# salesforce/LayoutDETR

Measured on AMD Instinct MI355X. Metric: images/sec G+D fwd-bwd, 256x256 bg x9 elems, higher is better.
Workload: dtype f32

## Files before the change

### include/ldetr_hip.h

```cpp
#ifndef LDETR_HIP_H
#define LDETR_HIP_H

#include <stdint.h>

#ifdef __cplusplus
extern "C" {
#endif

const char* ldetr_last_error(void);
int ldetr_abi_version(void);

int ldetr_debug_trace_tiles(int64_t* buffer);

int ldetr_set_split_bf16(int tiles);

int ldetr_engine_launch_counts(int64_t* f32_pipe, int64_t* bf16_split_pipe);

int ldetr_set_workspace(void* ptr, int64_t bytes);

typedef struct ldetr_tensor4 {
    int N, C, H, W;
    int64_t sn, sc, sh, sw;
} ldetr_tensor4;

typedef struct ldetr_epilogue {
    float alpha;
    const float* col_scale;
    const float* col_bias;
    const float* samp_scale;
    int64_t samp_ld;
    const float* residual;
    int64_t ldr;
    int act;
    float act_alpha;
    float act_gain;
    const float* mask_src;
    int64_t ldm;
    int mask_mode;
    float out_scale;
    float p_drop;
    uint64_t seed;
    const uint64_t* seed_ptr;
    int accumulate;
    float* a_rowsum;
} ldetr_epilogue;

int ldetr_bias_act_f32(const float* x, const float* b, const float* xref, const float* yref, const float* dy, float* y,
                       int64_t sizeX, int sizeB, int64_t stepB, int grad, int act, float alpha, float gain, float clamp,
                       void* stream);

int ldetr_upfirdn2d_f32(const float* x, const float* f, float* y, int N, int C, int inH, int inW,
                        const int64_t* x_strides_nchw, int fh, int fw, int64_t f_stride_h, int64_t f_stride_w,
                        int upx, int upy, int downx, int downy, int padx0, int padx1, int pady0, int pady1, int flip,
                        float gain, int outH, int outW, const int64_t* y_strides_nchw,
                        const float* act_bias, int has_act, float act_alpha, float act_gain, void* stream);

int ldetr_gemm_f32(const float* A, int64_t lda, int ta, const float* B, int64_t ldb, int tb, float* C, int64_t ldc,
                   int M, int N, int K, int splitk, const ldetr_epilogue* ep, int pix_per_sample, void* stream);

typedef struct ldetr_gemm_desc {
    const float* A; int64_t lda; int ta;
    const float* B; int64_t ldb; int tb;
    float* C; int64_t ldc;
    int M, N, K, splitk;
    const ldetr_epilogue* ep;
    int pix_per_sample;
} ldetr_gemm_desc;
int ldetr_gemm_pair_f32(const ldetr_gemm_desc* g0, const ldetr_gemm_desc* g1, void* stream);
int ldetr_gemm_pair_is_single_launch(const ldetr_gemm_desc* g0, const ldetr_gemm_desc* g1);

int ldetr_conv2d_fwd_f32(const float* x, const ldetr_tensor4* xt, const float* w, int Cout, int KH, int KW, int stride,
                         int pad, float* y, int64_t ldy, int OH, int OW, const float* in_scale, int64_t in_scale_ld,
                         const ldetr_epilogue* ep, void* stream);
int ldetr_conv2d_bwd_data_f32(const float* dy, const ldetr_tensor4* dyt, const float* w, int Cin, int KH, int KW,
                              int stride, int pad, float* dx, int64_t lddx, int IH, int IW, const float* dy_scale,
                              int64_t dy_scale_ld, const ldetr_epilogue* ep, void* stream);
int ldetr_conv2d_bwd_weight_f32(const float* x, const ldetr_tensor4* xt, const float* dy, const ldetr_tensor4* dyt,
                                float* dw, int KH, int KW, int stride, int pad, int splitk, const float* x_scale,
                                int64_t x_scale_ld, const float* dy_scale, int64_t dy_scale_ld, int accumulate, void* stream);

int ldetr_conv_transpose2d_fwd_f32(const float* x, const ldetr_tensor4* xt, const float* w, int Cout, int KH, int KW,
                                   int stride, int pad, float* y, int64_t ldy, int OH, int OW, const float* in_scale,
                                   int64_t in_scale_ld, const ldetr_epilogue* ep, void* stream);
int ldetr_conv_transpose2d_bwd_data_f32(const float* dy, const ldetr_tensor4* dyt, const float* w, int Cin, int KH,
                                        int KW, int stride, int pad, float* dx, int64_t lddx, int IH, int IW,
                                        const float* dy_scale, int64_t dy_scale_ld, const ldetr_epilogue* ep,
                                        void* stream);
int ldetr_conv_transpose2d_bwd_weight_f32(const float* x, const ldetr_tensor4* xt, const float* dy,
                                          const ldetr_tensor4* dyt, float* dw, int KH, int KW, int stride, int pad,
                                          int splitk, const float* x_scale, int64_t x_scale_ld, const float* dy_scale,
                                          int64_t dy_scale_ld, int accumulate, void* stream);

int ldetr_attention_fwd_f32(const float* q, int64_t ldq, const float* k, int64_t ldk, const float* v, int64_t ldv,
                            const unsigned char* key_padding_mask, float* out, int64_t ldo, float* lse, int B, int H,
                            int Lq, int Lk, int head_dim, float scale, float p_drop, uint64_t seed, const uint64_t* seed_ptr,
                            int causal, void* stream);
int ldetr_attention_bwd_f32(const float* q, int64_t ldq, const float* k, int64_t ldk, const float* v, int64_t ldv,
                            const unsigned char* key_padding_mask, const float* out, int64_t ldo, const float* lse,
                            const float* dout, int64_t lddo, float* dq, int64_t lddq, float* dk, int64_t lddk,
                            float* dv, int64_t lddv, int B, int H, int Lq, int Lk, int head_dim, float scale,
                            float p_drop, uint64_t seed, const uint64_t* seed_ptr, int causal, void* stream);

int ldetr_torgb_bwd_finish_f32(const float* dws, const float* s, const float* w, int B, int C, float* dw, float* ds, void* stream);

int ldetr_loss_combine_fwd_f32(const float* const* x, const float* w, const int* n, const int* fn, const int* red, int K, int ld,
                               float* vals, float* sums, float* total, void* stream);
int ldetr_loss_combine_bwd_f32(const float* const* x, const float* w, const int* n, const int* fn, const int* red, int K, int ld,
                               const float* g, float* grads, void* stream);
int ldetr_masked_mse_fwd_f32(const float* a, const float* b, const uint8_t* valid, int64_t rows, int D, int bdiv, float* out2, void* stream);
int ldetr_masked_mse_bwd_f32(const float* a, const float* b, const uint8_t* valid, int64_t rows, int D, int bdiv, const float* out2,
                             const float* g, float* da, void* stream);

typedef struct ldetr_ln_args {
    const float* x; const float* r; const float* gamma; const float* beta;
    float* y; float* z; float* mean; float* rstd;
    const float* dy; float* dx; float* dr; float* dgamma; float* dbeta;
    int64_t rows; int D; float eps, p_drop; uint64_t seed; const uint64_t* seed_ptr;
    const float* pos; int64_t pos_rows; float* ypos; const float* dy2;
    int r_parts; int64_t r_part_stride; const float* r_bias;
    const float* dy_parts; int dy_nparts; int64_t dy_part_stride;
} ldetr_ln_args;
int ldetr_layernorm_fwd_group_f32(const ldetr_ln_args* a, int n, void* stream);
int ldetr_layernorm_bwd_group_f32(const ldetr_ln_args* a, int n, void* stream);
int ldetr_sum_parts_f32(const float* base, const float* parts, int n_parts, int64_t part_stride, float* out, int64_t n, void* stream);

typedef struct ldetr_ffn_args {
    const float* x; int64_t ldx;
    const float* w1; const float* b1;
    const float* w2;
    float* h;
    float* ypart;
    int M, F;
    float p_drop; uint64_t seed; const uint64_t* seed_ptr;
    const float* dy;
    float* dxpart;
    float* dh;
} ldetr_ffn_args;
int ldetr_ffn_fwd_group_f32(const ldetr_ffn_args* a, int n, void* stream);
int ldetr_ffn_bwd_group_f32(const ldetr_ffn_args* a, int n, void* stream);

typedef struct ldetr_mha_small_args {
    const float* x; int64_t ldx;
    const float* w_in; const float* b_in; const float* w_out;
    const unsigned char* kpm;
    float* qkv; float* o; float* lse; float* ypart;
    int B, L;
    float scale, p_drop; uint64_t seed; const uint64_t* seed_ptr;
    const float* dr;
    float* dqkv; float* dxpart;
} ldetr_mha_small_args;
int ldetr_mha_small_fwd_group_f32(const ldetr_mha_small_args* a, int n, void* stream);
int ldetr_mha_small_bwd_group_f32(const ldetr_mha_small_args* a, int n, void* stream);

typedef struct ldetr_mha_cross_args {
    const float* x; int64_t ldx;
    const float* w_q; const float* b_q;
    const float* k; int64_t ldk; const float* v; int64_t ldv;
    const float* w_out;
    const unsigned char* kpm;
    float* q; float* o; float* lse; float* ypart;
    int B, Lq, Lk;
    float scale, p_drop; uint64_t seed; const uint64_t* seed_ptr;
    const float* dr;
    float* dq; float* dk; int64_t lddk; float* dv; int64_t lddv; float* dxpart;
} ldetr_mha_cross_args;
int ldetr_mha_cross_fwd_f32(const ldetr_mha_cross_args* a, void* stream);
int ldetr_mha_cross_bwd_f32(const ldetr_mha_cross_args* a, void* stream);

typedef struct ldetr_wgrad_desc {
    const float* A; int64_t lda; const float* B; int64_t ldb;
    float* dW; int64_t ldw; float* db;
    int M, rows, cols;
} ldetr_wgrad_desc;
int ldetr_wgrad_multi_f32(const ldetr_wgrad_desc* d, int n, void* stream);

int ldetr_colsum_f32(const float* a, float* red, int B, int64_t P, int C, void* stream);
int ldetr_act_bwd_reduce_f32(const float* dy, const float* y, float* dv, const float* bias, const float* demod,
                             float* dbias, float* ddemod, int B, int64_t P, int C, int act, float alpha, float gain,
                             void* stream);
int ldetr_mul_reduce_f32(const float* a, const float* x, const float* scale, float* out, float* red, int B, int64_t P,
                         int C, void* stream);
int ldetr_torgb_fwd_f32(const float* x, const float* w, const float* styles, const float* bias, float* y,
                        int B, int64_t P, int C, void* stream);
int ldetr_torgb_bwd_f32(const float* x, const float* dy, const float* w, const float* styles, float* dx, float* dws,
                        float* dbias, int B, int64_t P, int C, void* stream);

int ldetr_maxpool3x3s2_fwd_f32(const float* x, float* y, unsigned char* idx, int N, int H, int W, int C, void* stream);
int ldetr_maxpool3x3s2_bwd_f32(const float* dy, const unsigned char* idx, float* dx, int N, int H, int W, int C,
                               void* stream);

int ldetr_grad_sanitize_f32(float* g, int64_t n, float scale, float nan_value, float posinf, float neginf,
                            void* stream);
int ldetr_adam_step_f32(float* p, const float* g, float* m, float* v, int64_t n, int64_t step, float lr, float beta1,
                        float beta2, float eps, int fuse_sanitize, float gscale, float nan_value, float posinf,
                        float neginf, void* stream);
int ldetr_adam_ema_step_f32(float* p, const float* g, float* m, float* v, int64_t n, int64_t step, float lr, float beta1, float beta2,
                            float eps, int fuse_sanitize, float gscale, float nan_value, float posinf, float neginf,
                            float* p_ema, float ema_beta, void* stream);
int ldetr_ema_lerp_f32(float* p_ema, const float* p, int64_t n, float beta, void* stream);

int ldetr_softmax_xent_fwd_f32(const float* logits, int64_t ld, const int64_t* targets, float* row_lse, float* loss_sum, float* count,
                               int64_t rows, int V, int64_t ignore_index, float label_smoothing, void* stream);
int ldetr_softmax_xent_bwd_f32(const float* logits, int64_t ld, const int64_t* targets, const float* row_lse, const float* count,
                               const float* grad_out, float* dlogits, int64_t ldd, int64_t rows, int V, int64_t ignore_index,
                               float label_smoothing, void* stream);

int ldetr_embedding_fwd_f32(const float* weight, const float* pos, const int64_t* ids, float* out, int64_t n, int d, int V, int T,
                            void* stream);
int ldetr_embedding_bwd_f32(const float* dy, const int64_t* ids, float* dweight, int64_t n, int d, int V, int64_t padding_idx,
                            void* stream);

int ldetr_resample_coeffs(int in_size, int out_size, int32_t* bounds, int32_t* weights, int64_t weights_capacity, int* ksize_out);
int ldetr_resize_normalize_u8(const uint8_t* src, int64_t images, int H, int W, int out_h, int out_w, const int32_t* hbounds,
                              const int32_t* hweights, int hksize, const int32_t* vbounds, const int32_t* vweights, int vksize,
                              uint8_t* tmp, uint8_t* out_u8, float* out_chw, float mean0, float mean1, float mean2, float std0,
                              float std1, float std2, void* stream);

#define LDETR_PAGE_FILTER_BLUR 1
#define LDETR_PAGE_FILTER_EDGE 2
int ldetr_page_filter_u8(const uint8_t* src, uint8_t* dst, int64_t images, int H, int W, int kind, float radius, void* stream);

int ldetr_demod_fwd_f32(const float* weight, int64_t so, int64_t si, int64_t sh, int64_t sw, const float* styles, float* dcoefs,
                        float* w2, int B, int O, int I, int KH, int KW, float eps, void* stream);
int ldetr_demod_bwd_f32(const float* weight, int64_t so, int64_t si, int64_t sh, int64_t sw, const float* styles, const float* dcoefs,
                        const float* w2, const float* grad_dcoefs, float* dweight, int accumulate_dweight, float* dstyles, int B, int O,
                        int I, int KH, int KW, void* stream);

int ldetr_layout_losses_f32(const float* bbox, const float* bbox_ref, const uint8_t* valid, int B, int N, float* losses,
                            float* grads, void* stream);
int ldetr_layout_losses_bwd_f32(const float* grads, const float* grad_losses, int B, int N, float* dbbox, void* stream);

int ldetr_layout_finish_f32(const float* bbox_in, const int* num, const float* factors, const unsigned char* jitter, const unsigned char* mode,
                            float* bbox_out, float* overlap, float* alignment, int* order, int C, int K, int N, void* stream);

#define LDETR_FILTER_BILINEAR 0
#define LDETR_FILTER_LANCZOS 1
typedef struct ldetr_layout_raster_args {
    int struct_bytes;
    int B, N, S, nrow, n_colors, n_pages;
    const float* bbox;
    const uint8_t* valid;
    const int32_t* labels;
    const uint8_t* palette;
    const int32_t* page_wh;
    const uint8_t* pages;
    int64_t pages_bytes;
    const int64_t* page_table;
    const int32_t* page_index;
    const int32_t* coeffs;
    int64_t coeffs_len;
    const int64_t* cell_coeffs;
    int32_t* cells_dev;
    uint8_t* out;
} ldetr_layout_raster_args;
int ldetr_resample_coeffs_filter(int filter, int in_size, int out_size, int32_t* bounds, int32_t* weights, int64_t weights_capacity, int* ksize_out);
int ldetr_layout_raster_cell_size(int W, int H, int S, int* wn_out, int* hn_out);
int ldetr_layout_raster_u8(const ldetr_layout_raster_args* a, void* stream);

typedef struct ldetr_patch_resize_args {
    int struct_bytes;
    int n_jobs;
    const uint8_t* src0;
    int64_t src0_bytes;
    const uint8_t* src1;
    int64_t src1_bytes;
    uint8_t* dst;
    int64_t dst_bytes;
    const int64_t* jobs;
    const int32_t* tables;
    const int32_t* tables_host;
    int64_t tables_len;
    int32_t* jobs_dev;
} ldetr_patch_resize_args;
typedef struct ldetr_image_raster_args {
    int struct_bytes;
    int B, N, S, nrow;
    const float* bbox;
    const uint8_t* valid;
    const int32_t* rects;
    const int64_t* patch_off;
    const int64_t* page_off;
    const int32_t* page_wh;
    const uint8_t* pixels;
    int64_t pixels_bytes;
    const int32_t* coeffs;
    int64_t coeffs_len;
    const int64_t* cell_coeffs;
    int32_t* cells_dev;
    uint8_t* out;
} ldetr_image_raster_args;
int ldetr_patch_resize_u8(const ldetr_patch_resize_args* a, void* stream);
int ldetr_image_raster_u8(const ldetr_image_raster_args* a, void* stream);

int ldetr_lsap_f64(const double* cost, int batch, int n, int maximize, int* row_ind, int* col_ind, void* stream);

int ldetr_layoutnet_features_f32(const float* bbox, const int64_t* label, const uint8_t* padding_mask, const int* label_map, int map_len,
                                 const float* weights, int64_t weights_len, int num_label, int B, int N, float* out, void* stream);

int ldetr_layoutnet_forward_f32(const float* bbox, const int64_t* label, const uint8_t* padding_mask, const float* enc_weights,
                                int64_t enc_len, const float* dec_weights, int64_t dec_len, int num_label, int B, int N,
                                float* logit_disc, float* logit_cls, float* bbox_pred, float* features, void* stream);

int ldetr_feature_stats_f64(const float* x, int64_t n, int F, double* raw_mean, double* raw_cov, void* stream);

int ldetr_box_giou_pairwise_f32(const float* boxes1, const float* boxes2, int B, int N, int M, int cxcywh, float* iou, float* uni,
                                float* giou, double* cost, double cost_sign, void* stream);

int ldetr_bmm_strided_f32(const float* A, const int64_t* sa, const float* B, const int64_t* sb, float* C, const int64_t* sc,
                          int nb1, int nb2, int M, int N, int K, float alpha, void* stream);

int ldetr_p3_split_f32(const float* src, int64_t ld, void* dst, int64_t rows, int C, void* stream);
int ldetr_p3_merge_f32(const void* src, float* dst, int64_t ld, int64_t rows, int C, void* stream);
int ldetr_p3_weight_bwd(const float* w_ohwi, const float* o_scale, void* dst, int O, int KH, int KW, int I, void* stream);

int ldetr_p3_weight_prep(const int64_t* table_dev, int nconv, int total_blocks, void* stream);

typedef struct ldetr_p3_epilogue {
    float alpha;
    const float* col_scale;
    const float* col_bias;
    const void* residual_p3;
    const float* residual_f32;
    const void* relu_mask_p3;
    int relu;
} ldetr_p3_epilogue;

int ldetr_p3_conv2d_fwd(const void* x, int N, int H, int W, int Cin, const void* w, int Cout, int KH, int KW, int stride, int pad,
                        const ldetr_p3_epilogue* ep, void* out_p3, float* out_f32, void* stream);
int ldetr_p3_conv2d_fwd_dual(const void* x1, const void* x2, int N, int H, int W, int Cin, const void* w1, const void* w2, int Cout, int KH, int KW,
                             int stride, int pad, const ldetr_p3_epilogue* ep1, const ldetr_p3_epilogue* ep2, void* out1_p3, float* out1_f32,
                             void* out2_p3, float* out2_f32, void* stream);
int ldetr_p3_conv2d_bwd_data(const void* dy, int N, int OH, int OW, int Cout, const void* wb, int Cin, int KH, int KW, int stride, int pad,
                             int IH, int IW, const ldetr_p3_epilogue* ep, void* out_p3, float* out_f32, void* stream);
int ldetr_p3_conv2d_bwd_weight(const void* x, int N, int H, int W, int Cin, const void* dy, int Cout, int KH, int KW, int stride, int pad,
                               const float* dy_scale, float* dw, void* stream);
int ldetr_p3_conv2d_bwd_pair(const void* dy, int N, int OH, int OW, int Cout, const void* wb, const void* x, int Cin, int KH, int KW, int stride, int pad,
                             int IH, int IW, const ldetr_p3_epilogue* ep, void* dx_p3, float* dx_f32, const float* dy_scale, float* dw,
                             int* launches, void* stream);

int ldetr_struct_sizes(int32_t* out6);

int ldetr_p3_last_launch(int32_t* info10);

int ldetr_engine_last_launch(int32_t* info10);

#ifdef __cplusplus
}
#endif
#endif
```

### layoutdetr_amd/_lib.py

```python
import ctypes
import os
from ctypes import (POINTER, Structure, c_char_p, c_double, c_float, c_int, c_int64, c_ubyte, c_uint64, c_void_p)

_HERE = os.path.dirname(os.path.abspath(__file__))
ABI_VERSION = 25
LIB_PATH = os.environ.get('LDETR_LIB') or os.path.join(_HERE, 'lib', 'libldetr_hip.so')


class Tensor4(Structure):
    _fields_ = [('N', c_int), ('C', c_int), ('H', c_int), ('W', c_int),
                ('sn', c_int64), ('sc', c_int64), ('sh', c_int64), ('sw', c_int64)]


class GemmDesc(Structure):
    _fields_ = [('A', c_void_p), ('lda', c_int64), ('ta', c_int), ('B', c_void_p), ('ldb', c_int64), ('tb', c_int),
                ('C', c_void_p), ('ldc', c_int64), ('M', c_int), ('N', c_int), ('K', c_int), ('splitk', c_int),
                ('ep', c_void_p), ('pix_per_sample', c_int)]


class P3Epilogue(Structure):
    _fields_ = [('alpha', c_float), ('col_scale', c_void_p), ('col_bias', c_void_p), ('residual_p3', c_void_p),
                ('residual_f32', c_void_p), ('relu_mask_p3', c_void_p), ('relu', c_int)]


class Epilogue(Structure):
    _fields_ = [('alpha', c_float), ('col_scale', c_void_p), ('col_bias', c_void_p), ('samp_scale', c_void_p),
                ('samp_ld', c_int64), ('residual', c_void_p), ('ldr', c_int64), ('act', c_int),
                ('act_alpha', c_float), ('act_gain', c_float), ('mask_src', c_void_p), ('ldm', c_int64),
                ('mask_mode', c_int), ('out_scale', c_float), ('p_drop', c_float), ('seed', c_uint64),
                ('seed_ptr', c_void_p), ('accumulate', c_int), ('a_rowsum', c_void_p)]


class LnArgs(Structure):
    _fields_ = [('x', c_void_p), ('r', c_void_p), ('gamma', c_void_p), ('beta', c_void_p),
                ('y', c_void_p), ('z', c_void_p), ('mean', c_void_p), ('rstd', c_void_p),
                ('dy', c_void_p), ('dx', c_void_p), ('dr', c_void_p), ('dgamma', c_void_p), ('dbeta', c_void_p),
                ('rows', c_int64), ('D', c_int), ('eps', c_float), ('p_drop', c_float), ('seed', c_uint64), ('seed_ptr', c_void_p),
                ('pos', c_void_p), ('pos_rows', c_int64), ('ypos', c_void_p), ('dy2', c_void_p),
                ('r_parts', c_int), ('r_part_stride', c_int64), ('r_bias', c_void_p),
                ('dy_parts', c_void_p), ('dy_nparts', c_int), ('dy_part_stride', c_int64)]


class FfnArgs(Structure):
    _fields_ = [('x', c_void_p), ('ldx', c_int64), ('w1', c_void_p), ('b1', c_void_p), ('w2', c_void_p), ('h', c_void_p), ('ypart', c_void_p),
                ('M', c_int), ('F', c_int), ('p_drop', c_float), ('seed', c_uint64), ('seed_ptr', c_void_p),
                ('dy', c_void_p), ('dxpart', c_void_p), ('dh', c_void_p)]


class MhaSmallArgs(Structure):
    _fields_ = [('x', c_void_p), ('ldx', c_int64), ('w_in', c_void_p), ('b_in', c_void_p), ('w_out', c_void_p), ('kpm', c_void_p),
                ('qkv', c_void_p), ('o', c_void_p), ('lse', c_void_p), ('ypart', c_void_p), ('B', c_int), ('L', c_int),
                ('scale', c_float), ('p_drop', c_float), ('seed', c_uint64), ('seed_ptr', c_void_p),
                ('dr', c_void_p), ('dqkv', c_void_p), ('dxpart', c_void_p)]


class MhaCrossArgs(Structure):
    _fields_ = [('x', c_void_p), ('ldx', c_int64), ('w_q', c_void_p), ('b_q', c_void_p), ('k', c_void_p), ('ldk', c_int64), ('v', c_void_p), ('ldv', c_int64),
                ('w_out', c_void_p), ('kpm', c_void_p), ('q', c_void_p), ('o', c_void_p), ('lse', c_void_p), ('ypart', c_void_p),
                ('B', c_int), ('Lq', c_int), ('Lk', c_int), ('scale', c_float), ('p_drop', c_float), ('seed', c_uint64), ('seed_ptr', c_void_p),
                ('dr', c_void_p), ('dq', c_void_p), ('dk', c_void_p), ('lddk', c_int64), ('dv', c_void_p), ('lddv', c_int64), ('dxpart', c_void_p)]


class WgradDesc(Structure):
    _fields_ = [('A', c_void_p), ('lda', c_int64), ('B', c_void_p), ('ldb', c_int64), ('dW', c_void_p), ('ldw', c_int64), ('db', c_void_p),
                ('M', c_int), ('rows', c_int), ('cols', c_int)]


class LayoutRasterArgs(Structure):
    _fields_ = [('struct_bytes', c_int), ('B', c_int), ('N', c_int), ('S', c_int), ('nrow', c_int), ('n_colors', c_int), ('n_pages', c_int),
                ('bbox', c_void_p), ('valid', c_void_p), ('labels', c_void_p), ('palette', c_void_p), ('page_wh', c_void_p),
                ('pages', c_void_p), ('pages_bytes', c_int64), ('page_table', c_void_p), ('page_index', c_void_p),
                ('coeffs', c_void_p), ('coeffs_len', c_int64), ('cell_coeffs', c_void_p), ('cells_dev', c_void_p), ('out', c_void_p)]


class PatchResizeArgs(Structure):
    _fields_ = [('struct_bytes', c_int), ('n_jobs', c_int), ('src0', c_void_p), ('src0_bytes', c_int64), ('src1', c_void_p), ('src1_bytes', c_int64),
                ('dst', c_void_p), ('dst_bytes', c_int64), ('jobs', c_void_p), ('tables', c_void_p), ('tables_host', c_void_p), ('tables_len', c_int64),
                ('jobs_dev', c_void_p)]


class ImageRasterArgs(Structure):
    _fields_ = [('struct_bytes', c_int), ('B', c_int), ('N', c_int), ('S', c_int), ('nrow', c_int),
                ('bbox', c_void_p), ('valid', c_void_p), ('rects', c_void_p), ('patch_off', c_void_p), ('page_off', c_void_p), ('page_wh', c_void_p),
                ('pixels', c_void_p), ('pixels_bytes', c_int64), ('coeffs', c_void_p), ('coeffs_len', c_int64), ('cell_coeffs', c_void_p),
                ('cells_dev', c_void_p), ('out', c_void_p)]


_P = c_void_p
_I = c_int
_L = c_int64
_F = c_float
_T4 = POINTER(Tensor4)
_EP = POINTER(Epilogue)

SIGNATURES = {
    'ldetr_set_workspace': [_P, _L],
    'ldetr_bias_act_f32': [_P, _P, _P, _P, _P, _P, _L, _I, _L, _I, _I, _F, _F, _F, _P],
    'ldetr_upfirdn2d_f32': [_P, _P, _P, _I, _I, _I, _I, POINTER(c_int64), _I, _I, _L, _L, _I, _I, _I, _I, _I, _I, _I, _I,
                            _I, _F, _I, _I, POINTER(c_int64), _P, _I, _F, _F, _P],
    'ldetr_gemm_f32': [_P, _L, _I, _P, _L, _I, _P, _L, _I, _I, _I, _I, _EP, _I, _P],
    'ldetr_conv2d_fwd_f32': [_P, _T4, _P, _I, _I, _I, _I, _I, _P, _L, _I, _I, _P, _L, _EP, _P],
    'ldetr_conv2d_bwd_data_f32': [_P, _T4, _P, _I, _I, _I, _I, _I, _P, _L, _I, _I, _P, _L, _EP, _P],
    'ldetr_conv2d_bwd_weight_f32': [_P, _T4, _P, _T4, _P, _I, _I, _I, _I, _I, _P, _L, _P, _L, _I, _P],
    'ldetr_conv_transpose2d_fwd_f32': [_P, _T4, _P, _I, _I, _I, _I, _I, _P, _L, _I, _I, _P, _L, _EP, _P],
    'ldetr_conv_transpose2d_bwd_data_f32': [_P, _T4, _P, _I, _I, _I, _I, _I, _P, _L, _I, _I, _P, _L, _EP, _P],
    'ldetr_conv_transpose2d_bwd_weight_f32': [_P, _T4, _P, _T4, _P, _I, _I, _I, _I, _I, _P, _L, _P, _L, _I, _P],
    'ldetr_attention_fwd_f32': [_P, _L, _P, _L, _P, _L, _P, _P, _L, _P, _I, _I, _I, _I, _I, _F, _F, c_uint64, _P, _I, _P],
    'ldetr_attention_bwd_f32': [_P, _L, _P, _L, _P, _L, _P, _P, _L, _P, _P, _L, _P, _L, _P, _L, _P, _L,
                                _I, _I, _I, _I, _I, _F, _F, c_uint64, _P, _I, _P],
    'ldetr_colsum_f32': [_P, _P, _I, _L, _I, _P],
    'ldetr_act_bwd_reduce_f32': [_P, _P, _P, _P, _P, _P, _P, _I, _L, _I, _I, _F, _F, _P],
    'ldetr_mul_reduce_f32': [_P, _P, _P, _P, _P, _I, _L, _I, _P],
    'ldetr_torgb_fwd_f32': [_P, _P, _P, _P, _P, _I, _L, _I, _P],
    'ldetr_torgb_bwd_f32': [_P, _P, _P, _P, _P, _P, _P, _I, _L, _I, _P],
    'ldetr_maxpool3x3s2_fwd_f32': [_P, _P, _P, _I, _I, _I, _I, _P],
    'ldetr_maxpool3x3s2_bwd_f32': [_P, _P, _P, _I, _I, _I, _I, _P],
    'ldetr_grad_sanitize_f32': [_P, _L, _F, _F, _F, _F, _P],
    'ldetr_adam_step_f32': [_P, _P, _P, _P, _L, _L, _F, _F, _F, _F, _I, _F, _F, _F, _F, _P],
    'ldetr_adam_ema_step_f32': [_P, _P, _P, _P, _L, _L, _F, _F, _F, _F, _I, _F, _F, _F, _F, _P, _F, _P],
    'ldetr_ema_lerp_f32': [_P, _P, _L, _F, _P],
    'ldetr_lsap_f64': [_P, _I, _I, _I, _P, _P, _P],
    'ldetr_layoutnet_features_f32': [_P, _P, _P, POINTER(c_int), _I, _P, _L, _I, _I, _I, _P, _P],
    'ldetr_layoutnet_forward_f32': [_P, _P, _P, _P, _L, _P, _L, _I, _I, _I, _P, _P, _P, _P, _P],
    'ldetr_feature_stats_f64': [_P, _L, _I, _P, _P, _P],
    'ldetr_box_giou_pairwise_f32': [_P, _P, _I, _I, _I, _I, _P, _P, _P, _P, c_double, _P],
    'ldetr_bmm_strided_f32': [_P, _P, _P, _P, _P, _P, _I, _I, _I, _I, _I, _F, _P],
    'ldetr_softmax_xent_fwd_f32': [_P, _L, _P, _P, _P, _P, _L, _I, _L, _F, _P],
    'ldetr_softmax_xent_bwd_f32': [_P, _L, _P, _P, _P, _P, _P, _L, _L, _I, _L, _F, _P],
    'ldetr_embedding_fwd_f32': [_P, _P, _P, _P, _L, _I, _I, _I, _P],
    'ldetr_embedding_bwd_f32': [_P, _P, _P, _L, _I, _I, _L, _P],
    'ldetr_debug_trace_tiles': [_P],
    'ldetr_set_split_bf16': [c_int],
    'ldetr_engine_launch_counts': [POINTER(c_int64), POINTER(c_int64)],
    'ldetr_layernorm_fwd_group_f32': [_P, _I, _P],
    'ldetr_layernorm_bwd_group_f32': [_P, _I, _P],
    'ldetr_sum_parts_f32': [_P, _P, _I, _L, _P, _L, _P],
    'ldetr_ffn_fwd_group_f32': [_P, _I, _P],
    'ldetr_ffn_bwd_group_f32': [_P, _I, _P],
    'ldetr_mha_small_fwd_group_f32': [_P, _I, _P],
    'ldetr_mha_small_bwd_group_f32': [_P, _I, _P],
    'ldetr_mha_cross_fwd_f32': [_P, _P],
    'ldetr_mha_cross_bwd_f32': [_P, _P],
    'ldetr_wgrad_multi_f32': [_P, _I, _P],
    'ldetr_loss_combine_fwd_f32': [_P, _P, _P, _P, _P, _I, _I, _P, _P, _P, _P],
    'ldetr_loss_combine_bwd_f32': [_P, _P, _P, _P, _P, _I, _I, _P, _P, _P],
    'ldetr_masked_mse_fwd_f32': [_P, _P, _P, _L, _I, _I, _P, _P],
    'ldetr_masked_mse_bwd_f32': [_P, _P, _P, _L, _I, _I, _P, _P, _P, _P],
    'ldetr_torgb_bwd_finish_f32': [_P, _P, _P, _I, _I, _P, _P, _P],
    'ldetr_gemm_pair_f32': [_P, _P, _P],
    'ldetr_gemm_pair_is_single_launch': [_P, _P],
    'ldetr_demod_fwd_f32': [_P, _L, _L, _L, _L, _P, _P, _P, _I, _I, _I, _I, _I, _F, _P],
    'ldetr_demod_bwd_f32': [_P, _L, _L, _L, _L, _P, _P, _P, _P, _P, _I, _P, _I, _I, _I, _I, _I, _P],
    'ldetr_layout_losses_f32': [_P, _P, _P, _I, _I, _P, _P, _P],
    'ldetr_layout_losses_bwd_f32': [_P, _P, _I, _I, _P, _P],
    'ldetr_layout_finish_f32': [_P, _P, _P, _P, _P, _P, _P, _P, _P, _I, _I, _I, _P],
    'ldetr_resample_coeffs': [_I, _I, _P, _P, _L, _P],
    'ldetr_resample_coeffs_filter': [_I, _I, _I, _P, _P, _L, _P],
    'ldetr_layout_raster_cell_size': [_I, _I, _I, _P, _P],
    'ldetr_layout_raster_u8': [_P, _P],
    'ldetr_patch_resize_u8': [_P, _P],
    'ldetr_image_raster_u8': [_P, _P],
    'ldetr_p3_split_f32': [_P, _L, _P, _L, _I, _P],
    'ldetr_p3_merge_f32': [_P, _P, _L, _L, _I, _P],
    'ldetr_p3_weight_bwd': [_P, _P, _P, _I, _I, _I, _I, _P],
    'ldetr_p3_conv2d_bwd_data': [_P, _I, _I, _I, _I, _P, _I, _I, _I, _I, _I, _I, _I, _P, _P, _P, _P],
    'ldetr_p3_conv2d_fwd': [_P, _I, _I, _I, _I, _P, _I, _I, _I, _I, _I, _P, _P, _P, _P],
    'ldetr_p3_conv2d_bwd_weight': [_P, _I, _I, _I, _I, _P, _I, _I, _I, _I, _I, _P, _P, _P],
    'ldetr_p3_weight_prep': [_P, _I, _I, _P],
    'ldetr_p3_conv2d_fwd_dual': [_P, _P, _I, _I, _I, _I, _P, _P, _I, _I, _I, _I, _I, _P, _P, _P, _P, _P, _P, _P],
    'ldetr_p3_conv2d_bwd_pair': [_P, _I, _I, _I, _I, _P, _P, _I, _I, _I, _I, _I, _I, _I, _P, _P, _P, _P, _P, _P, _P],
    'ldetr_p3_last_launch': [_P],
    'ldetr_engine_last_launch': [_P],
    'ldetr_struct_sizes': [_P],
    'ldetr_resize_normalize_u8': [_P, _L, _I, _I, _I, _I, _P, _P, _I, _P, _P, _I, _P, _P, _P, _F, _F, _F, _F, _F, _F, _P],
    'ldetr_page_filter_u8': [_P, _P, _L, _I, _I, _I, _F, _P],
}

_lib = None


def load():
    global _lib
    if _lib is not None:
        return _lib
    if not os.path.exists(LIB_PATH):
        raise RuntimeError(
            f'{LIB_PATH} not found: build the gfx950 kernels first (python -m layoutdetr_amd.build or '
            f'__graft_entry__.build()).  layoutdetr_amd has no CPU/PyTorch fallback path.')
    import torch
    lib = ctypes.CDLL(LIB_PATH)
    lib.ldetr_last_error.restype = c_char_p
    lib.ldetr_last_error.argtypes = []
    lib.ldetr_abi_version.restype = c_int
    lib.ldetr_abi_version.argtypes = []
    for name, argtypes in SIGNATURES.items():
        fn = getattr(lib, name)
        fn.restype = c_int
        fn.argtypes = argtypes
    if lib.ldetr_abi_version() != ABI_VERSION:
        raise RuntimeError('libldetr_hip.so ABI version mismatch; rebuild it')
    sizes = (ctypes.c_int32 * 6)()
    lib.ldetr_struct_sizes(sizes)
    mirror = [ctypes.sizeof(t) for t in (LnArgs, FfnArgs, MhaSmallArgs, MhaCrossArgs, WgradDesc, P3Epilogue)]
    if list(sizes) != mirror:
        raise RuntimeError(f'libldetr_hip.so argument blocks {list(sizes)} do not match the ctypes mirror {mirror}; rebuild')
    _lib = lib
    return lib


def check(rc, what=''):
    if rc != 0:
        msg = load().ldetr_last_error().decode('utf-8', 'replace')
        raise RuntimeError(f'{what}: {msg}' if what else msg)
```

### layoutdetr_amd/build.py

```python
import hashlib
import os
import shutil
import subprocess
import sys
from concurrent.futures import ThreadPoolExecutor

HERE = os.path.dirname(os.path.abspath(__file__))
CSRC = os.path.join(HERE, 'csrc')
LIBDIR = os.path.join(HERE, 'lib')
OBJDIR = os.path.join(LIBDIR, 'obj')
LIBNAME = 'libldetr_hip.so'
ARCH = 'gfx950'

SOURCES = ['ldetr_core.cpp', 'bias_act.hip', 'upfirdn2d.hip', 'gemm_conv.hip', 'attention.hip', 'layernorm.hip',
           'misc_ops.hip', 'optim.hip', 'lsap.hip', 'xent.hip', 'resample.hip', 'layout_loss.hip', 'demod.hip', 'wgrad_smallc.hip', 'stem_conv.hip', 'box_ops.hip', 'ffn_fused.hip', 'conv_c32.hip', 'mha_small.hip', 'p3_engine.hip', 'bmm_strided.hip', 'layoutnet.hip', 'layoutnet_train.hip', 'layout_finish.hip', 'layout_raster.hip', 'page_filter.hip', 'patch_resize.hip']
HEADERS = ['ldetr_common.hpp', 'layoutnet_layers.hpp', os.path.join('..', '..', 'include', 'ldetr_hip.h')]

FLAGS = ([] if os.environ.get('LDETR_TILE_TRACE') else ['-DLDETR_TILE_TRACE=0']) + (['-DP3_TRACE'] if os.environ.get('LDETR_P3_TRACE') else []) + ['-O3', '-std=c++17', '-fPIC', f'--offload-arch={ARCH}', '-munsafe-fp-atomics', '-fno-gpu-rdc',
         '-Wno-unused-result', '-Rpass-analysis=kernel-resource-usage']
NO_SCRATCH = ('wgrad_c32_3x3_kernel', 'gemm_f32_kernel', 'gemm_small_kernel', 'attn_fwd_kernel', 'attn_fwd_wide_kernel', 'attn_bwd_kernel', 'ffn_fwd_kernel', 'ffn_bwd_kernel', 'conv3x3_c32_kernel', 'mha_small_fwd_kernel', 'mha_cross_fwd_kernel', 'mha_small_bwd_kernel', 'mha_cross_bwd_kernel', 'wgrad_multi_kernel', 'ln_fwd_kernel', 'ln_bwd_kernel', 'p3_nt_kernel', 'p3_tn_kernel', 'p3_c3_kernel', 'p3_bwd_pair', 'layoutnet_features_kernel', 'layoutnet_forward_kernel', 'feature_stats_f64_kernel', 'layout_finish_kernel', 'layout_raster_kernel', 'page_blur_kernel', 'page_edge_kernel', 'patch_resize_kernel')


def _hipcc():
    for cand in (os.environ.get('HIPCC'), shutil.which('hipcc'), '/opt/rocm/bin/hipcc'):
        if cand and os.path.exists(cand):
            return cand
    raise RuntimeError('hipcc not found: the gfx950 kernel library cannot be built')


def _digest(paths):
    h = hashlib.sha256()
    for p in paths:
        with open(p, 'rb') as f:
            h.update(f.read())
    h.update(' '.join(FLAGS).encode())
    return h.hexdigest()


def _kernel_resources(remarks):
    out, cur = {}, None
    for line in remarks.splitlines():
        if 'remark:' not in line:
            continue
        body = line.split('remark:', 1)[1].split('[-Rpass-analysis', 1)[0].strip()
        if body.startswith('Function Name:'):
            cur = body.split(':', 1)[1].strip()
            out[cur] = {}
        elif cur is not None and ':' in body:
            k, v = body.rsplit(':', 1)
            out[cur][k.strip()] = v.strip()
    return out


def source_digest():
    return _digest(sorted(os.path.join(CSRC, f) for f in os.listdir(CSRC) if f.endswith(('.hip', '.cpp', '.hpp')) and not f.startswith('.'))
                   + [os.path.normpath(os.path.join(CSRC, HEADERS[-1]))])


def lib_path():
    return os.path.join(LIBDIR, LIBNAME)


def build(force=False, verbose=True):
    os.makedirs(OBJDIR, exist_ok=True)
    hipcc = _hipcc()
    hdrs = [os.path.normpath(os.path.join(CSRC, h)) for h in HEADERS]
    objs, jobs = [], []
    for src in SOURCES:
        sp = os.path.join(CSRC, src)
        obj = os.path.join(OBJDIR, src + '.o')
        stamp = obj + '.sha'
        dig = _digest([sp] + hdrs)
        objs.append(obj)
        if not force and os.path.exists(obj) and os.path.exists(stamp) and open(stamp).read() == dig:
            continue
        jobs.append((sp, obj, stamp, dig))

    def compile_one(job):
        sp, obj, stamp, dig = job
        cmd = [hipcc] + FLAGS + ['-x', 'hip', '-c', sp, '-o', obj]
        if verbose:
            print('[ldetr build]', os.path.basename(sp), flush=True)
        r = subprocess.run(cmd, capture_output=True, text=True)
        if r.returncode != 0:
            raise RuntimeError(f'hipcc failed for {sp}:\n{r.stdout}\n{r.stderr}')
        res = _kernel_resources(r.stderr)
        with open(obj + '.resources.txt', 'w') as f:
            for name, d in res.items():
                f.write(f"{name} vgprs={d.get('VGPRs', '?')} agprs={d.get('AGPRs', '?')} scratch={d.get('ScratchSize [bytes/lane]', '?')} "
                        f"occupancy={d.get('Occupancy [waves/SIMD]', '?')} lds={d.get('LDS Size [bytes/block]', '?')}\n")
        bad = [n for n, d in res.items() if any(k in n for k in NO_SCRATCH) and d.get('ScratchSize [bytes/lane]', '0') != '0']
        if bad:
            raise RuntimeError(f'{os.path.basename(sp)}: scratch memory in register-budgeted kernels: ' + ', '.join(bad[:4]))
        with open(stamp, 'w') as f:
            f.write(dig)

    if jobs:
        with ThreadPoolExecutor(max_workers=min(8, len(jobs))) as ex:
            list(ex.map(compile_one, jobs))
    out = lib_path()
    if jobs or not os.path.exists(out):
        cmd = [hipcc, '-shared', '-fPIC', f'--offload-arch={ARCH}', '-fno-gpu-rdc', '-o', out] + objs
        r = subprocess.run(cmd, capture_output=True, text=True)
        if r.returncode != 0:
            raise RuntimeError(f'link failed:\n{r.stdout}\n{r.stderr}')
        if verbose:
            print('[ldetr build] linked', out, flush=True)
    return out


if __name__ == '__main__':
    build(force='--force' in sys.argv)
```

### layoutdetr_amd/csrc/misc_ops.hip

```cpp
#include "ldetr_common.hpp"
#include "../../include/ldetr_hip.h"

namespace ldetr {

enum { RR_COLSUM = 0, RR_ACTGRAD = 1, RR_MULRED = 2 };

struct RRParams {
    const float* a; const float* b; float* out;
    const float* colv;
    const float* sampv;
    float* red1; long red1_bs;
    float* red2; long red2_bs;
    float* part;
    long P; int B, C, mode, act, rows_pb;
    float alpha, gain;
};

template <int MODE>
__global__ __launch_bounds__(256) void rowreduce_kernel(RRParams p) {
    __shared__ float4 sh1[256];
    __shared__ float4 sh2[256];
    const int C4 = p.C >> 2;
    const int TQ = C4 < 256 ? C4 : 256;
    const int RL = 256 / TQ;
    const int tx = threadIdx.x % TQ, ty = threadIdx.x / TQ;
    const int cq = blockIdx.z * TQ + tx;
    const int b = blockIdx.y;
    const bool active = (ty < RL) && (cq < C4);
    float4 r1 = make_float4(0.f, 0.f, 0.f, 0.f), r2 = r1;
    if (active) {
        const int c = cq << 2;
        float4 cv = make_float4(0.f, 0.f, 0.f, 0.f), sv = make_float4(1.f, 1.f, 1.f, 1.f);
        if (p.colv) cv = *reinterpret_cast<const float4*>(p.colv + c);
        if (p.sampv) sv = *reinterpret_cast<const float4*>(p.sampv + (long)b * p.C + c);
        const long r0 = (long)blockIdx.x * p.rows_pb;
        const long r1e = min(p.P, r0 + p.rows_pb);
        auto process = [&](const float4& a, const float4& x2, long off) {
            if (MODE == RR_COLSUM) {
                r1.x += a.x; r1.y += a.y; r1.z += a.z; r1.w += a.w;
            } else if (MODE == RR_ACTGRAD) {
                const float4& y = x2;
                float4 dv;
                float gp = p.gain, gn = (p.act == 2) ? p.gain * p.alpha : (p.act == 1 ? 0.f : p.gain);
                dv.x = a.x * (y.x > 0.f ? gp : gn); dv.y = a.y * (y.y > 0.f ? gp : gn);
                dv.z = a.z * (y.z > 0.f ? gp : gn); dv.w = a.w * (y.w > 0.f ? gp : gn);
                if (p.out) *reinterpret_cast<float4*>(p.out + off) = dv;
                r1.x += dv.x; r1.y += dv.y; r1.z += dv.z; r1.w += dv.w;
                if (p.red2) {
                    float ip = 1.f / gp, in = (gn != 0.f) ? 1.f / gn : 0.f;
                    float vx = y.x * (y.x > 0.f ? ip : in) - cv.x, vy = y.y * (y.y > 0.f ? ip : in) - cv.y;
                    float vz = y.z * (y.z > 0.f ? ip : in) - cv.z, vw = y.w * (y.w > 0.f ? ip : in) - cv.w;
                    r2.x += dv.x * vx / sv.x; r2.y += dv.y * vy / sv.y; r2.z += dv.z * vz / sv.z; r2.w += dv.w * vw / sv.w;
                }
            } else {
                if (p.out) {
                    float4 o = make_float4(a.x * sv.x, a.y * sv.y, a.z * sv.z, a.w * sv.w);
                    *reinterpret_cast<float4*>(p.out + off) = o;
                }
                r1.x += a.x * x2.x; r1.y += a.y * x2.y; r1.z += a.z * x2.z; r1.w += a.w * x2.w;
            }
        };
        constexpr int UN = 4;
        for (long r = r0 + ty; r < r1e; r += (long)RL * UN) {
            float4 av[UN], bv[UN];
#pragma unroll
            for (int u = 0; u < UN; u++) {
                const long rr = r + (long)u * RL;
                if (rr < r1e) {
                    const long off = ((long)b * p.P + rr) * p.C + c;
                    av[u] = *reinterpret_cast<const float4*>(p.a + off);
                    if (MODE != RR_COLSUM) bv[u] = *reinterpret_cast<const float4*>(p.b + off);
                }
            }
#pragma unroll
            for (int u = 0; u < UN; u++) {
                const long rr = r + (long)u * RL;
                if (rr < r1e) process(av[u], bv[u], ((long)b * p.P + rr) * p.C + c);
            }
        }
    }
    sh1[threadIdx.x] = r1; sh2[threadIdx.x] = r2;
    __syncthreads();
    if (active && ty == 0) {
        for (int j = 1; j < RL; j++) {
            float4 t = sh1[j * TQ + tx]; r1.x += t.x; r1.y += t.y; r1.z += t.z; r1.w += t.w;
            float4 u = sh2[j * TQ + tx]; r2.x += u.x; r2.y += u.y; r2.z += u.z; r2.w += u.w;
        }
        const int c = cq << 2;
        if (p.part) {
            const long nblk = (long)gridDim.x * gridDim.y, blk = (long)blockIdx.y * gridDim.x + blockIdx.x;
            *reinterpret_cast<float4*>(p.part + blk * p.C + c) = r1;
            if (p.red2) *reinterpret_cast<float4*>(p.part + (nblk + blk) * p.C + c) = r2;
            return;
        }
        if (p.red1) {
            float* d = p.red1 + (long)b * p.red1_bs + c;
            atomicAdd(d, r1.x); atomicAdd(d + 1, r1.y); atomicAdd(d + 2, r1.z); atomicAdd(d + 3, r1.w);
        }
        if (p.red2) {
            float* d = p.red2 + (long)b * p.red2_bs + c;
            atomicAdd(d, r2.x); atomicAdd(d + 1, r2.y); atomicAdd(d + 2, r2.z); atomicAdd(d + 3, r2.w);
        }
    }
}

__global__ __launch_bounds__(256) void rr_finish_kernel(RRParams p, int chunks, int segs) {
    __shared__ float sh[256];
    const int which = blockIdx.z / segs, seg = blockIdx.z % segs;
    float* red = which ? p.red2 : p.red1;
    const long bs = which ? p.red2_bs : p.red1_bs;
    if (!red) return;
    const bool shared_by_batch = bs == 0;
    if (shared_by_batch && blockIdx.y > 0) return;
    const int c = blockIdx.x * 64 + (threadIdx.x & 63), lane = threadIdx.x >> 6;
    const long nblk = (long)chunks * p.B;
    const float* part = p.part + (which ? nblk * p.C : 0);
    const long first = shared_by_batch ? 0 : (long)blockIdx.y * chunks, count = shared_by_batch ? nblk : chunks;
    const long per = (count + segs - 1) / segs, i0 = seg * per, i1 = min(count, i0 + per);
    float acc = 0.f;
    if (c < p.C) {
#pragma unroll 4
        for (long i = i0 + lane; i < i1; i += 4) acc += part[(first + i) * p.C + c];
    }
    sh[threadIdx.x] = acc;
    __syncthreads();
    if (lane == 0 && c < p.C && i0 < i1) {
        acc += sh[threadIdx.x + 64] + sh[threadIdx.x + 128] + sh[threadIdx.x + 192];
        float* d = red + (shared_by_batch ? 0 : (long)blockIdx.y * bs) + c;
        if (segs > 1) atomicAdd(d, acc); else *d += acc;
    }
}

static int launch_rr(RRParams& p, hipStream_t st) {
    const int C4 = p.C / 4;
    const int TQ = C4 < 256 ? C4 : 256;
    const int RL = 256 / TQ;
    static const long target = 2048;
    const long groups = (long)p.B * cdiv(C4, TQ);
    long chunks = target / groups; if (chunks < 1) chunks = 1;
    long rows_pb = (p.P + chunks - 1) / chunks;
    const long min_rows = (long)RL * 4;
    if (rows_pb < min_rows) rows_pb = min_rows;
    rows_pb = (rows_pb + RL - 1) / RL * RL;
    p.rows_pb = (int)rows_pb;
    dim3 grid((unsigned)((p.P + rows_pb - 1) / rows_pb), p.B, cdiv(C4, TQ));
    const long nblk = (long)grid.x * grid.y;
    const long sharers = p.red1 && p.red1_bs == 0 ? nblk : (long)grid.x;
    p.part = (p.red1 || p.red2) && sharers > 32 ? scratch_alloc((size_t)nblk * p.C * sizeof(float) * (p.red2 ? 2 : 1)) : nullptr;
    if (p.mode == RR_COLSUM) hipLaunchKernelGGL(rowreduce_kernel<RR_COLSUM>, grid, 256, 0, st, p);
    else if (p.mode == RR_ACTGRAD) hipLaunchKernelGGL(rowreduce_kernel<RR_ACTGRAD>, grid, 256, 0, st, p);
    else hipLaunchKernelGGL(rowreduce_kernel<RR_MULRED>, grid, 256, 0, st, p);
    int rc = check_launch("rowreduce"); if (rc || !p.part) return rc;
    int segs = (int)(sharers / 32); if (segs < 1) segs = 1; if (segs > 16) segs = 16;
    hipLaunchKernelGGL(rr_finish_kernel, dim3(cdiv(p.C, 64), p.B, (p.red2 ? 2 : 1) * segs), 256, 0, st, p, (int)grid.x, segs);
    return check_launch("rowreduce_finish");
}

struct PoolParams {
    const float* x; float* y; unsigned char* idx; const float* dy; float* dx;
    int N, H, W, C, OH, OW;
};

__global__ __launch_bounds__(256) void maxpool_fwd_kernel(PoolParams p) {
    const int C4 = p.C >> 2;
    const long total = (long)p.N * p.OH * p.OW * C4;
    for (long i = (long)blockIdx.x * blockDim.x + threadIdx.x; i < total; i += (long)gridDim.x * blockDim.x) {
        int c = (int)(i % C4) << 2; long t = i / C4;
        int ox = (int)(t % p.OW); t /= p.OW;
        int oy = (int)(t % p.OH); int n = (int)(t / p.OH);
        float4 m = make_float4(-INFINITY, -INFINITY, -INFINITY, -INFINITY);
        uchar4 mi = make_uchar4(0, 0, 0, 0);
#pragma unroll
        for (int kh = 0; kh < 3; kh++) {
            int y = oy * 2 - 1 + kh;
            if (y < 0 || y >= p.H) continue;
#pragma unroll
            for (int kw = 0; kw < 3; kw++) {
                int x = ox * 2 - 1 + kw;
                if (x < 0 || x >= p.W) continue;
                float4 v = *reinterpret_cast<const float4*>(p.x + (((long)n * p.H + y) * p.W + x) * p.C + c);
                unsigned char k = (unsigned char)(kh * 3 + kw);
                if (v.x > m.x || v.x != v.x) { m.x = v.x; mi.x = k; }
                if (v.y > m.y || v.y != v.y) { m.y = v.y; mi.y = k; }
                if (v.z > m.z || v.z != v.z) { m.z = v.z; mi.z = k; }
                if (v.w > m.w || v.w != v.w) { m.w = v.w; mi.w = k; }
            }
        }
        long o = (((long)n * p.OH + oy) * p.OW + ox) * p.C + c;
        *reinterpret_cast<float4*>(p.y + o) = m;
        if (p.idx) *reinterpret_cast<uchar4*>(p.idx + o) = mi;
    }
}

__global__ __launch_bounds__(256) void maxpool_bwd_kernel(PoolParams p) {
    const int C4 = p.C >> 2;
    const long total = (long)p.N * p.H * p.W * C4;
    for (long i = (long)blockIdx.x * blockDim.x + threadIdx.x; i < total; i += (long)gridDim.x * blockDim.x) {
        int c = (int)(i % C4) << 2; long t = i / C4;
        int x = (int)(t % p.W); t /= p.W;
        int y = (int)(t % p.H); int n = (int)(t / p.H);
        float4 g = make_float4(0.f, 0.f, 0.f, 0.f);
        int oy0 = y >> 1, oy1 = (y + 1) >> 1;
        int ox0 = x >> 1, ox1 = (x + 1) >> 1;
        for (int oy = oy0; oy <= oy1; oy++) {
            if (oy >= p.OH) continue;
            for (int ox = ox0; ox <= ox1; ox++) {
                if (ox >= p.OW) continue;
                unsigned char k = (unsigned char)((y - (oy * 2 - 1)) * 3 + (x - (ox * 2 - 1)));
                long o = (((long)n * p.OH + oy) * p.OW + ox) * p.C + c;
                uchar4 mi = *reinterpret_cast<const uchar4*>(p.idx + o);
                float4 d = *reinterpret_cast<const float4*>(p.dy + o);
                if (mi.x == k) g.x += d.x;
                if (mi.y == k) g.y += d.y;
                if (mi.z == k) g.z += d.z;
                if (mi.w == k) g.w += d.w;
            }
        }
        *reinterpret_cast<float4*>(p.dx + (((long)n * p.H + y) * p.W + x) * p.C + c) = g;
    }
}

struct RgbParams {
    const float* x; const float* dy; const float* w; const float* s;
    float* dx; float* dws; float* dbias;
    long P; int B, C, rows_pb;
};

__global__ __launch_bounds__(256) void torgb_bwd_kernel(RgbParams p) {
    __shared__ float4 sh[3][256];
    const int C4 = p.C >> 2;
    const int TQ = C4 < 256 ? C4 : 256;
    const int RL = 256 / TQ;
    const int tx = threadIdx.x % TQ, ty = threadIdx.x / TQ;
    const int cq = blockIdx.z * TQ + tx;
    const int b = blockIdx.y;
    const bool active = (ty < RL) && (cq < C4);
    float4 a0 = make_float4(0.f, 0.f, 0.f, 0.f), a1 = a0, a2 = a0;
    float db0 = 0.f, db1 = 0.f, db2 = 0.f;
    if (active) {
        const int c = cq << 2;
        const float4 w0 = *reinterpret_cast<const float4*>(p.w + c);
        const float4 w1 = *reinterpret_cast<const float4*>(p.w + p.C + c);
        const float4 w2 = *reinterpret_cast<const float4*>(p.w + 2 * p.C + c);
        const float4 sv = *reinterpret_cast<const float4*>(p.s + (long)b * p.C + c);
        const long r0 = (long)blockIdx.x * p.rows_pb;
        const long r1e = min(p.P, r0 + p.rows_pb);
        for (long r = r0 + ty; r < r1e; r += RL) {
            const long row = (long)b * p.P + r;
            const float d0 = p.dy[row * 3], d1 = p.dy[row * 3 + 1], d2 = p.dy[row * 3 + 2];
            const float4 xv = *reinterpret_cast<const float4*>(p.x + row * p.C + c);
            float4 o;
            o.x = sv.x * (d0 * w0.x + d1 * w1.x + d2 * w2.x); o.y = sv.y * (d0 * w0.y + d1 * w1.y + d2 * w2.y);
            o.z = sv.z * (d0 * w0.z + d1 * w1.z + d2 * w2.z); o.w = sv.w * (d0 * w0.w + d1 * w1.w + d2 * w2.w);
            *reinterpret_cast<float4*>(p.dx + row * p.C + c) = o;
            a0.x += d0 * xv.x; a0.y += d0 * xv.y; a0.z += d0 * xv.z; a0.w += d0 * xv.w;
            a1.x += d1 * xv.x; a1.y += d1 * xv.y; a1.z += d1 * xv.z; a1.w += d1 * xv.w;
            a2.x += d2 * xv.x; a2.y += d2 * xv.y; a2.z += d2 * xv.z; a2.w += d2 * xv.w;
            if (cq == 0) { db0 += d0; db1 += d1; db2 += d2; }
        }
    }
    sh[0][threadIdx.x] = a0; sh[1][threadIdx.x] = a1; sh[2][threadIdx.x] = a2;
    __syncthreads();
    if (active && ty == 0) {
        for (int j = 1; j < RL; j++) {
            float4 t0 = sh[0][j * TQ + tx], t1 = sh[1][j * TQ + tx], t2 = sh[2][j * TQ + tx];
            a0.x += t0.x; a0.y += t0.y; a0.z += t0.z; a0.w += t0.w;
            a1.x += t1.x; a1.y += t1.y; a1.z += t1.z; a1.w += t1.w;
            a2.x += t2.x; a2.y += t2.y; a2.z += t2.z; a2.w += t2.w;
        }
        const int c = cq << 2;
        float* d = p.dws + (long)b * 3 * p.C + c;
        atomicAdd(d, a0.x); atomicAdd(d + 1, a0.y); atomicAdd(d + 2, a0.z); atomicAdd(d + 3, a0.w);
        d += p.C;
        atomicAdd(d, a1.x); atomicAdd(d + 1, a1.y); atomicAdd(d + 2, a1.z); atomicAdd(d + 3, a1.w);
        d += p.C;
        atomicAdd(d, a2.x); atomicAdd(d + 1, a2.y); atomicAdd(d + 2, a2.z); atomicAdd(d + 3, a2.w);
    }
    if (p.dbias && blockIdx.z == 0) {
        __syncthreads();
        float* f = reinterpret_cast<float*>(&sh[0][0]);
        if (tx == 0 && ty < RL) { f[ty * 3] = db0; f[ty * 3 + 1] = db1; f[ty * 3 + 2] = db2; }
        __syncthreads();
        if (threadIdx.x < 3) {
            float t = 0.f;
            for (int j = 0; j < RL; j++) t += f[j * 3 + threadIdx.x];
            atomicAdd(p.dbias + threadIdx.x, t);
        }
    }
}

__global__ __launch_bounds__(256) void torgb_finish_kernel(const float* __restrict__ dws, const float* __restrict__ s, const float* __restrict__ w,
                                                           float* __restrict__ dw, float* __restrict__ ds, int B, int C) {
    const int i = blockIdx.x * 256 + threadIdx.x;
    if (i < 3 * C) {
        const int c = i % C;
        float a = 0.f;
        for (int b = 0; b < B; b++) a += dws[(long)b * 3 * C + i] * s[(long)b * C + c];
        dw[i] += a;
    }
    if (i < B * C) {
        const int b = i / C, c = i - b * C;
        const float* d = dws + (long)b * 3 * C + c;
        ds[i] = d[0] * w[c] + d[C] * w[C + c] + d[2 * C] * w[2 * C + c];
    }
}

}

using namespace ldetr;

static int rr_common(RRParams& p, const char* what) {
    LDETR_CHECK(p.a, "%s: null pointer", what);
    LDETR_CHECK(p.C % 4 == 0 && p.C > 0, "%s: C must be a positive multiple of 4", what);
    LDETR_CHECK(p.B > 0 && p.P >= 0, "%s: bad shape", what);
    return LDETR_OK;
}

extern "C" int ldetr_colsum_f32(const float* a, float* red, int B, int64_t P, int C, void* stream) {
    RRParams p; memset(&p, 0, sizeof(p));
    p.a = a; p.red1 = red; p.red1_bs = C; p.B = B; p.P = P; p.C = C; p.mode = RR_COLSUM;
    int rc = rr_common(p, "colsum"); if (rc) return rc;
    if (P == 0) return LDETR_OK;
    return launch_rr(p, (hipStream_t)stream);
}

extern "C" int ldetr_act_bwd_reduce_f32(const float* dy, const float* y, float* dv, const float* bias, const float* demod,
                                        float* dbias, float* ddemod, int B, int64_t P, int C, int act, float alpha, float gain,
                                        void* stream) {
    RRParams p; memset(&p, 0, sizeof(p));
    p.a = dy; p.b = y; p.out = dv; p.colv = bias; p.sampv = demod; p.red1 = dbias; p.red1_bs = 0;
    p.red2 = ddemod; p.red2_bs = C; p.B = B; p.P = P; p.C = C; p.mode = RR_ACTGRAD; p.act = act; p.alpha = alpha; p.gain = gain;
    int rc = rr_common(p, "act_bwd_reduce"); if (rc) return rc;
    LDETR_CHECK(y, "act_bwd_reduce: y is required");
    LDETR_CHECK(!ddemod || demod, "act_bwd_reduce: ddemod needs demod");
    if (P == 0) return LDETR_OK;
    return launch_rr(p, (hipStream_t)stream);
}

extern "C" int ldetr_mul_reduce_f32(const float* a, const float* x, const float* scale, float* out, float* red,
                                    int B, int64_t P, int C, void* stream) {
    RRParams p; memset(&p, 0, sizeof(p));
    p.a = a; p.b = x; p.out = out; p.sampv = scale; p.red1 = red; p.red1_bs = C; p.B = B; p.P = P; p.C = C; p.mode = RR_MULRED;
    int rc = rr_common(p, "mul_reduce"); if (rc) return rc;
    LDETR_CHECK(x, "mul_reduce: x is required");
    if (P == 0) return LDETR_OK;
    return launch_rr(p, (hipStream_t)stream);
}

extern "C" int ldetr_maxpool3x3s2_fwd_f32(const float* x, float* y, unsigned char* idx, int N, int H, int W, int C, void* stream) {
    LDETR_CHECK(x && y, "maxpool_fwd: null pointer");
    LDETR_CHECK(C % 4 == 0, "maxpool_fwd: C must be a multiple of 4");
    PoolParams p; memset(&p, 0, sizeof(p));
    p.x = x; p.y = y; p.idx = idx; p.N = N; p.H = H; p.W = W; p.C = C; p.OH = (H + 2 - 3) / 2 + 1; p.OW = (W + 2 - 3) / 2 + 1;
    long total = (long)N * p.OH * p.OW * (C / 4);
    int grid = (int)((total + 255) / 256); if (grid > 8192) grid = 8192; if (grid < 1) grid = 1;
    hipLaunchKernelGGL(maxpool_fwd_kernel, grid, 256, 0, (hipStream_t)stream, p);
    return check_launch("maxpool_fwd");
}

extern "C" int ldetr_maxpool3x3s2_bwd_f32(const float* dy, const unsigned char* idx, float* dx, int N, int H, int W, int C, void* stream) {
    LDETR_CHECK(dy && idx && dx, "maxpool_bwd: null pointer");
    LDETR_CHECK(C % 4 == 0, "maxpool_bwd: C must be a multiple of 4");
    PoolParams p; memset(&p, 0, sizeof(p));
    p.dy = dy; p.idx = const_cast<unsigned char*>(idx); p.dx = dx; p.N = N; p.H = H; p.W = W; p.C = C;
    p.OH = (H + 2 - 3) / 2 + 1; p.OW = (W + 2 - 3) / 2 + 1;
    long total = (long)N * H * W * (C / 4);
    int grid = (int)((total + 255) / 256); if (grid > 8192) grid = 8192; if (grid < 1) grid = 1;
    hipLaunchKernelGGL(maxpool_bwd_kernel, grid, 256, 0, (hipStream_t)stream, p);
    return check_launch("maxpool_bwd");
}

namespace ldetr {
struct RgbFwdParams { const float* x; const float* w; const float* s; const float* bias; float* y; long P; int B, C; };

template <int LPP>
__global__ __launch_bounds__(256) void torgb_fwd_kernel(RgbFwdParams p) {
    const int lane_in = threadIdx.x % LPP;
    const long pix_per_block = 256 / LPP;
    const int C4 = p.C >> 2;
    const int b = blockIdx.y;
    const float* sb = p.s + (long)b * p.C;
    float4 w0[2], w1[2], w2[2];
#pragma unroll
    for (int t = 0; t < 2; t++) {
        const int cq = lane_in + t * LPP;
        if (cq < C4) {
            const float4 sv = *reinterpret_cast<const float4*>(sb + 4 * cq);
            float4 a = *reinterpret_cast<const float4*>(p.w + 4 * cq), bq = *reinterpret_cast<const float4*>(p.w + p.C + 4 * cq), c = *reinterpret_cast<const float4*>(p.w + 2 * p.C + 4 * cq);
            w0[t] = make_float4(a.x * sv.x, a.y * sv.y, a.z * sv.z, a.w * sv.w);
            w1[t] = make_float4(bq.x * sv.x, bq.y * sv.y, bq.z * sv.z, bq.w * sv.w);
            w2[t] = make_float4(c.x * sv.x, c.y * sv.y, c.z * sv.z, c.w * sv.w);
        } else { w0[t] = w1[t] = w2[t] = make_float4(0.f, 0.f, 0.f, 0.f); }
    }
    const float b0 = p.bias ? p.bias[0] : 0.f, b1 = p.bias ? p.bias[1] : 0.f, b2 = p.bias ? p.bias[2] : 0.f;
    const long stride = (long)gridDim.x * pix_per_block;
    for (long r = (long)blockIdx.x * pix_per_block + threadIdx.x / LPP; r < p.P; r += stride) {
        const float* xr = p.x + ((long)b * p.P + r) * p.C;
        float d0 = 0.f, d1 = 0.f, d2 = 0.f;
#pragma unroll
        for (int t = 0; t < 2; t++) {
            const int cq = lane_in + t * LPP;
            if (cq < C4) {
                const float4 xv = *reinterpret_cast<const float4*>(xr + 4 * cq);
                d0 += xv.x * w0[t].x + xv.y * w0[t].y + xv.z * w0[t].z + xv.w * w0[t].w;
                d1 += xv.x * w1[t].x + xv.y * w1[t].y + xv.z * w1[t].z + xv.w * w1[t].w;
                d2 += xv.x * w2[t].x + xv.y * w2[t].y + xv.z * w2[t].z + xv.w * w2[t].w;
            }
        }
#pragma unroll
        for (int o = LPP / 2; o > 0; o >>= 1) { d0 += __shfl_xor(d0, o, 64); d1 += __shfl_xor(d1, o, 64); d2 += __shfl_xor(d2, o, 64); }
        if (lane_in == 0) {
            float* yr = p.y + ((long)b * p.P + r) * 3;
            yr[0] = d0 + b0; yr[1] = d1 + b1; yr[2] = d2 + b2;
        }
    }
}
}

extern "C" int ldetr_torgb_fwd_f32(const float* x, const float* w, const float* styles, const float* bias, float* y,
                                   int B, int64_t P, int C, void* stream) {
    LDETR_CHECK(x && w && styles && y, "torgb_fwd: null pointer");
    const int C4 = C / 4;
    LDETR_CHECK(C % 4 == 0 && C4 >= 1 && C <= 512 && (C4 & (C4 - 1)) == 0, "torgb_fwd: C must be 4 x a power of two, at most 512 (got %d)", C);
    LDETR_CHECK((((uintptr_t)x | (uintptr_t)w | (uintptr_t)styles) & 15) == 0, "torgb_fwd: buffers must be 16-byte aligned");
    if (B == 0 || P == 0) return LDETR_OK;
    RgbFwdParams p; p.x = x; p.w = w; p.s = styles; p.bias = bias; p.y = y; p.P = P; p.B = B; p.C = C;
    const int lpp = C4 < 64 ? C4 : 64;
    const long ppb = 256 / lpp;
    long gx = (P + ppb - 1) / ppb; if (gx > 4096) gx = 4096;
    const dim3 grid((unsigned)gx, (unsigned)B);
    hipStream_t st = (hipStream_t)stream;
    switch (lpp) {
        case 1: hipLaunchKernelGGL(torgb_fwd_kernel<1>, grid, 256, 0, st, p); break;
        case 2: hipLaunchKernelGGL(torgb_fwd_kernel<2>, grid, 256, 0, st, p); break;
        case 4: hipLaunchKernelGGL(torgb_fwd_kernel<4>, grid, 256, 0, st, p); break;
        case 8: hipLaunchKernelGGL(torgb_fwd_kernel<8>, grid, 256, 0, st, p); break;
        case 16: hipLaunchKernelGGL(torgb_fwd_kernel<16>, grid, 256, 0, st, p); break;
        case 32: hipLaunchKernelGGL(torgb_fwd_kernel<32>, grid, 256, 0, st, p); break;
        default: hipLaunchKernelGGL(torgb_fwd_kernel<64>, grid, 256, 0, st, p); break;
    }
    return check_launch("torgb_fwd");
}

extern "C" int ldetr_torgb_bwd_f32(const float* x, const float* dy, const float* w, const float* styles,
                                   float* dx, float* dws, float* dbias, int B, int64_t P, int C, void* stream) {
    LDETR_CHECK(x && dy && w && styles && dx && dws, "torgb_bwd: null pointer");
    LDETR_CHECK(C % 4 == 0, "torgb_bwd: C must be a multiple of 4");
    RgbParams p; memset(&p, 0, sizeof(p));
    p.x = x; p.dy = dy; p.w = w; p.s = styles; p.dx = dx; p.dws = dws; p.dbias = dbias; p.B = B; p.P = P; p.C = C;
    const int C4 = C / 4; const int TQ = C4 < 256 ? C4 : 256; const int RL = 256 / TQ;
    long rows_pb = (long)RL * 16;
    long nb = ((P + rows_pb - 1) / rows_pb) * B * cdiv(C4, TQ);
    while (nb > 2048) { rows_pb *= 2; nb = ((P + rows_pb - 1) / rows_pb) * B * cdiv(C4, TQ); }
    p.rows_pb = (int)rows_pb;
    dim3 grid((unsigned)((P + rows_pb - 1) / rows_pb), B, cdiv(C4, TQ));
    hipLaunchKernelGGL(torgb_bwd_kernel, grid, 256, 0, (hipStream_t)stream, p);
    return check_launch("torgb_bwd");
}

extern "C" int ldetr_torgb_bwd_finish_f32(const float* dws, const float* s, const float* w, int B, int C, float* dw, float* ds, void* stream) {
    LDETR_CHECK(dws && s && w && dw && ds && B > 0 && C > 0, "torgb_bwd_finish: bad arguments");
    const int n = (B > 3 ? B : 3) * C;
    hipLaunchKernelGGL(torgb_finish_kernel, dim3((unsigned)((n + 255) / 256)), 256, 0, (hipStream_t)stream, dws, s, w, dw, ds, B, C);
    return check_launch("torgb_bwd_finish");
}
```

### layoutdetr_amd/hip/modconv.py

```python
import ctypes
import math

import torch

from . import core
from .conv import weight_ohwi, _grad_to_oihw
from .core import ACT_LRELU, ACT_NONE
from .linear import act_backward
from ..torch_utils.ops import upfirdn2d as _up


def _mul_reduce(a, x, scale, B, P, C, want_out=True):
    out = torch.empty_like(a) if want_out else None
    red = core.zeros((B, C), a.device)
    core.check(core.lib().ldetr_mul_reduce_f32(core.ptr(a), core.ptr(x), core.ptr(scale), core.ptr(out), core.ptr(red),
                                               B, P, C, core.stream()), 'mul_reduce')
    return out, red


def _prescaled_for_wgrad(x, dv, s, d, B, H):
    if B >= 8 and H <= 16:
        return x * s[:, None, None, :], dv * d[:, None, None, :], None, None
    return x, dv, s, d


class _ModConvFn(torch.autograd.Function):

    @staticmethod
    def forward(ctx, x, weight, styles, dcoefs, bias, pad, act_alpha, act_gain):
        core.require_gpu(x, weight, styles, dcoefs, bias)
        x = core.f32c(x); w = core.f32c(weight_ohwi(weight)); s = core.f32c(styles); d = core.f32c(dcoefs); b = core.f32c(bias)
        B, H, W, I = x.shape
        O, KH, KW, _ = w.shape
        OH, OW = H + 2 * pad - KH + 1, W + 2 * pad - KW + 1
        y = torch.empty((B, OH, OW, O), device=x.device, dtype=torch.float32)
        xt = core.tensor4_nhwc(x)
        ep = core.epilogue(samp_scale=d, col_bias=b, act=ACT_LRELU, act_alpha=act_alpha, act_gain=act_gain)
        core.engine_call('ldetr_conv2d_fwd_f32', 2.0 * B * OH * OW * O * KH * KW * I, lambda: core.check(core.lib().ldetr_conv2d_fwd_f32(core.ptr(x), ctypes.byref(xt), core.ptr(w), O, KH, KW, 1, pad, core.ptr(y), O,
                                                   OH, OW, core.ptr(s), s.stride(0), ctypes.byref(ep), core.stream()), 'modconv_fwd'), operands=(x, y, w))
        ctx.save_for_backward(x, w, s, d, b, y)
        ctx.cfg = (pad, act_alpha, act_gain)
        ctx.params = (weight, bias)
        return y

    @staticmethod
    def backward(ctx, dy):
        x, w, s, d, b, y = ctx.saved_tensors
        pad, act_alpha, act_gain = ctx.cfg
        B, H, W, I = x.shape
        O, KH, KW, _ = w.shape
        _, OH, OW, _ = y.shape
        dy = core.f32c(dy)
        wparam, bparam = ctx.params
        dv2, dbias, ddemod = act_backward(dy.reshape(-1, O), y.reshape(-1, O), ACT_LRELU, act_alpha, act_gain, True,
                                          bias=b, demod=d, want_ddemod=True, B=B, dbias_out=core.flat_grad(bparam))
        dv = dv2.reshape(B, OH, OW, O)
        dvt = core.tensor4_nhwc(dv)
        dx = dw = ds = None
        if ctx.needs_input_grad[0] or ctx.needs_input_grad[2]:
            dxs = torch.empty((B, H, W, I), device=dy.device, dtype=torch.float32)
            core.engine_call('ldetr_conv2d_bwd_data_f32', 2.0 * B * OH * OW * O * KH * KW * I, lambda: core.check(core.lib().ldetr_conv2d_bwd_data_f32(core.ptr(dv), ctypes.byref(dvt), core.ptr(w), I, KH, KW, 1, pad,
                                                            core.ptr(dxs), I, H, W, core.ptr(d), d.stride(0), None, core.stream()),
                       'modconv_bwd_data'), operands=(dv, dxs, w))
            dx, ds = _mul_reduce(dxs, x, s, B, H * W, I)
        if ctx.needs_input_grad[1]:
            gw = core.flat_grad(wparam)
            acc = 0
            if gw is not None and gw.permute(0, 2, 3, 1).is_contiguous():
                dw_ohwi, acc = gw.permute(0, 2, 3, 1), 1
            else:
                dw_ohwi = torch.empty((O, KH, KW, I), device=dy.device, dtype=torch.float32)
            sk = 0
            xw, dvw, sw, dw_ = _prescaled_for_wgrad(x, dv, s, d, B, H)
            xwt, dvwt = core.tensor4_nhwc(xw), core.tensor4_nhwc(dvw)
            core.engine_call('ldetr_conv2d_bwd_weight_f32', 2.0 * B * OH * OW * O * KH * KW * I, lambda: core.check(core.lib().ldetr_conv2d_bwd_weight_f32(core.ptr(xw), ctypes.byref(xwt), core.ptr(dvw), ctypes.byref(dvwt),
                                                              core.ptr(dw_ohwi), KH, KW, 1, pad, sk, core.ptr(sw), sw.stride(0) if sw is not None else 0,
                                                              core.ptr(dw_), dw_.stride(0) if dw_ is not None else 0, acc, core.stream()), 'modconv_bwd_weight'), operands=(x, dv, dw_ohwi))
            dw = None if acc else _grad_to_oihw(dw_ohwi)
        return dx, dw, ds, ddemod, dbias, None, None, None


class _ModConvUpFn(torch.autograd.Function):

    @staticmethod
    def forward(ctx, x, weight, styles, dcoefs, bias, f, act_alpha, act_gain):
        core.require_gpu(x, weight, styles, dcoefs, bias, f)
        x = core.f32c(x); w = core.f32c(weight_ohwi(weight)); s = core.f32c(styles); d = core.f32c(dcoefs); b = core.f32c(bias)
        B, H, W, I = x.shape
        O, KH, KW, _ = w.shape
        UH, UW = (H - 1) * 2 + KH, (W - 1) * 2 + KW
        ud = torch.empty((B, UH, UW, O), device=x.device, dtype=torch.float32)
        xt = core.tensor4_nhwc(x)
        ep = core.epilogue(samp_scale=d)
        core.engine_call('ldetr_conv_transpose2d_fwd_f32', 2.0 * B * H * W * O * KH * KW * I, lambda: core.check(core.lib().ldetr_conv_transpose2d_fwd_f32(core.ptr(x), ctypes.byref(xt), core.ptr(w), O, KH, KW, 2, 0, core.ptr(ud),
                                                             O, UH, UW, core.ptr(s), s.stride(0), ctypes.byref(ep), core.stream()),
                   'modconv_up_fwd'), operands=(x, ud, w))
        y = _up._kernel_call(ud.permute(0, 3, 1, 2), f, 1, 1, 1, 1, 1, 1, 1, 1, False, 4.0, act_bias=b,
                             act=(act_alpha, act_gain)).permute(0, 2, 3, 1)
        ctx.save_for_backward(x, w, s, d, b, f, ud, y)
        ctx.cfg = (act_alpha, act_gain)
        ctx.params = (weight, bias)
        return y

    @staticmethod
    def backward(ctx, dy):
        x, w, s, d, b, f, ud, y = ctx.saved_tensors
        act_alpha, act_gain = ctx.cfg
        B, H, W, I = x.shape
        O, KH, KW, _ = w.shape
        _, UH, UW, _ = ud.shape
        dy = core.f32c(dy)
        wparam, bparam = ctx.params
        dv2, dbias, _ = act_backward(dy.reshape(-1, O), y.reshape(-1, O), ACT_LRELU, act_alpha, act_gain, True,
                                     dbias_out=core.flat_grad(bparam))
        dv = dv2.reshape(y.shape)
        dud = _up._kernel_call(dv.permute(0, 3, 1, 2), f, 1, 1, 1, 1, 2, 2, 2, 2, True, 4.0).permute(0, 2, 3, 1)
        _, dd_num = _mul_reduce(dud, ud, None, B, UH * UW, O, want_out=False)
        ddemod = dd_num / d
        dudt = core.tensor4_nhwc(dud)
        dx = dw = ds = None
        if ctx.needs_input_grad[0] or ctx.needs_input_grad[2]:
            dxs = torch.empty((B, H, W, I), device=dy.device, dtype=torch.float32)
            core.engine_call('ldetr_conv_transpose2d_bwd_data_f32', 2.0 * B * H * W * O * KH * KW * I, lambda: core.check(core.lib().ldetr_conv_transpose2d_bwd_data_f32(core.ptr(dud), ctypes.byref(dudt), core.ptr(w), I, KH, KW, 2, 0,
                                                                      core.ptr(dxs), I, H, W, core.ptr(d), d.stride(0), None,
                                                                      core.stream()), 'modconv_up_bwd_data'), operands=(dud, dxs, w))
            dx, ds = _mul_reduce(dxs, x, s, B, H * W, I)
        if ctx.needs_input_grad[1]:
            gw = core.flat_grad(wparam)
            acc = 0
            if gw is not None and gw.permute(0, 2, 3, 1).is_contiguous():
                dw_ohwi, acc = gw.permute(0, 2, 3, 1), 1
            else:
                dw_ohwi = torch.empty((O, KH, KW, I), device=dy.device, dtype=torch.float32)
            sk = 0
            xw, dudw, sw, dw_ = _prescaled_for_wgrad(x, dud, s, d, B, H)
            xwt, dudwt = core.tensor4_nhwc(xw), core.tensor4_nhwc(dudw)
            core.engine_call('ldetr_conv_transpose2d_bwd_weight_f32', 2.0 * B * H * W * O * KH * KW * I, lambda: core.check(core.lib().ldetr_conv_transpose2d_bwd_weight_f32(core.ptr(xw), ctypes.byref(xwt), core.ptr(dudw), ctypes.byref(dudwt),
                                                                        core.ptr(dw_ohwi), KH, KW, 2, 0, sk, core.ptr(sw), sw.stride(0) if sw is not None else 0,
                                                                        core.ptr(dw_), dw_.stride(0) if dw_ is not None else 0, acc, core.stream()), 'modconv_up_bwd_weight'), operands=(x, dud, dw_ohwi))
            dw = None if acc else _grad_to_oihw(dw_ohwi)
        return dx, dw, ds, ddemod, dbias, None, None, None


class _ToRGBFn(torch.autograd.Function):

    @staticmethod
    def forward(ctx, x, weight, styles, bias):
        core.require_gpu(x, weight, styles, bias)
        x = core.f32c(x); s = core.f32c(styles); b = core.f32c(bias)
        w = core.f32c(weight.reshape(weight.shape[0], -1))
        B, H, W, C = x.shape
        O = w.shape[0]
        y = torch.empty((B, H, W, O), device=x.device, dtype=torch.float32)
        c4 = C // 4
        if O == 3 and C % 4 == 0 and C <= 512 and (c4 & (c4 - 1)) == 0 and s.stride(0) == C:
            core.check(core.lib().ldetr_torgb_fwd_f32(core.ptr(x), core.ptr(w), core.ptr(s), core.ptr(b), core.ptr(y), B, H * W, C, core.stream()), 'torgb_fwd')
        else:
            xt = core.tensor4_nhwc(x)
            ep = core.epilogue(col_bias=b)
            core.engine_call('ldetr_conv2d_fwd_f32', 2.0 * B * H * W * O * C, lambda: core.check(core.lib().ldetr_conv2d_fwd_f32(core.ptr(x), ctypes.byref(xt), core.ptr(w), O, 1, 1, 1, 0, core.ptr(y), O, H, W,
                                                       core.ptr(s), s.stride(0), ctypes.byref(ep), core.stream()), 'torgb_fwd'), operands=(x, y, w))
        ctx.save_for_backward(x, w, s)
        ctx.wshape = weight.shape
        ctx.params = (weight, bias)
        return y

    @staticmethod
    def backward(ctx, dy):
        x, w, s = ctx.saved_tensors
        B, H, W, C = x.shape
        O = w.shape[0]
        if O != 3:
            raise NotImplementedError('toRGB backward kernel is specialised for 3 colour channels')
        dy = core.f32c(dy)
        dx = torch.empty_like(x)
        dws = core.zeros((B, O, C), x.device)
        wparam, bparam = ctx.params
        gw, gb = core.flat_grad(wparam), core.flat_grad(bparam)
        gw = gw.reshape(O, C) if (gw is not None and gw.is_contiguous()) else None
        dbias = gb if gb is not None else torch.zeros(O, device=x.device, dtype=torch.float32)
        dw = gw if gw is not None else torch.zeros((O, C), device=x.device, dtype=torch.float32)
        ds = torch.empty((B, C), device=x.device, dtype=torch.float32)
        core.check(core.lib().ldetr_torgb_bwd_f32(core.ptr(x), core.ptr(dy), core.ptr(w), core.ptr(s), core.ptr(dx), core.ptr(dws),
                                                  core.ptr(dbias), B, H * W, C, core.stream()), 'torgb_bwd')
        core.check(core.lib().ldetr_torgb_bwd_finish_f32(core.ptr(dws), core.ptr(s), core.ptr(w), B, C, core.ptr(dw), core.ptr(ds), core.stream()), 'torgb_bwd_finish')
        return dx, (None if gw is not None else dw.reshape(ctx.wshape)), ds, (None if gb is not None else dbias)


class _DemodFn(torch.autograd.Function):

    @staticmethod
    def forward(ctx, weight, styles):
        core.require_gpu(weight, styles)
        w = weight.detach()
        if w.dtype != torch.float32:
            w = w.float()
        s = core.f32c(styles.detach())
        O, I, KH, KW = w.shape
        B = s.shape[0]
        d = torch.empty((B, O), device=s.device, dtype=torch.float32)
        w2 = torch.empty((O, I), device=s.device, dtype=torch.float32)
        st = w.stride()
        core.check(core.lib().ldetr_demod_fwd_f32(core.ptr(w), st[0], st[1], st[2], st[3], core.ptr(s), core.ptr(d), core.ptr(w2),
                                                  B, O, I, KH, KW, 1e-8, core.stream()), 'demod_fwd')
        ctx.save_for_backward(w, s, d, w2)
        ctx.wparam = weight
        return d

    @staticmethod
    def backward(ctx, g):
        w, s, d, w2 = ctx.saved_tensors
        O, I, KH, KW = w.shape
        B = s.shape[0]
        g = core.f32c(g)
        need_w, need_s = ctx.needs_input_grad
        acc = core.flat_grad(ctx.wparam) if need_w else None
        accumulate = acc is not None and acc.stride() == w.stride()
        dw = acc if accumulate else (torch.empty_strided(w.shape, w.stride(), device=w.device, dtype=torch.float32) if need_w else None)
        ds = torch.empty_like(s) if need_s else None
        st = w.stride()
        core.check(core.lib().ldetr_demod_bwd_f32(core.ptr(w), st[0], st[1], st[2], st[3], core.ptr(s), core.ptr(d), core.ptr(w2), core.ptr(g),
                                                  core.ptr(dw), 1 if accumulate else 0, core.ptr(ds), B, O, I, KH, KW, core.stream()), 'demod_bwd')
        return (None if accumulate else dw), ds


def demod_coefs(weight, styles):
    if styles.shape[0] > 64:
        from .linear import linear
        return (linear(styles.square(), weight.square().sum(dim=[2, 3])) + 1e-8).rsqrt()
    return _DemodFn.apply(weight, styles)


def modconv3x3(x, weight, styles, bias, act_alpha=0.2, act_gain=math.sqrt(2)):
    d = demod_coefs(weight, styles)
    return _ModConvFn.apply(x, weight, styles, d, bias, weight.shape[2] // 2, act_alpha, act_gain)


def modconv3x3_up2(x, weight, styles, bias, f, act_alpha=0.2, act_gain=math.sqrt(2)):
    d = demod_coefs(weight, styles)
    return _ModConvUpFn.apply(x, weight, styles, d, bias, f, act_alpha, act_gain)


def torgb(x, weight, styles, bias):
    return _ToRGBFn.apply(x, weight, styles, bias)
```

### layoutdetr_amd/training/networks_stylegan2.py

```python
import math

import numpy as np
import torch

from ..hip import core, modconv
from ..hip.linear import linear
from ..torch_utils.ops import bias_act, upfirdn2d


def normalize_2nd_moment(x, dim=1, eps=1e-8):
    return x * (x.square().mean(dim=dim, keepdim=True) + eps).rsqrt()


class FullyConnectedLayer(torch.nn.Module):
    def __init__(self, in_features, out_features, bias=True, activation='linear', lr_multiplier=1, bias_init=0):
        super().__init__()
        self.in_features = in_features
        self.out_features = out_features
        self.activation = activation
        self.weight = torch.nn.Parameter(torch.randn([out_features, in_features]) / lr_multiplier)
        self.bias = torch.nn.Parameter(torch.full([out_features], np.float32(bias_init))) if bias else None
        self.weight_gain = lr_multiplier / np.sqrt(in_features)
        self.bias_gain = lr_multiplier

    def forward(self, x):
        b = self.bias
        spec = bias_act.activation_funcs[self.activation]
        if self.activation == 'lrelu' and b is not None and self.bias_gain != 1 and self.bias_gain > 0:
            return linear(x, self.weight, b, act=core.ACT_LRELU, act_alpha=float(spec.def_alpha), act_gain=float(spec.def_gain * self.bias_gain),
                          wscale=float(self.weight_gain / self.bias_gain))
        if b is not None and self.bias_gain != 1:
            b = b * self.bias_gain
        if self.activation == 'linear':
            return linear(x, self.weight, b, wscale=float(self.weight_gain))
        if self.activation in ('relu', 'lrelu'):
            act = core.ACT_RELU if self.activation == 'relu' else core.ACT_LRELU
            return linear(x, self.weight, b, act=act, act_alpha=float(spec.def_alpha), act_gain=float(spec.def_gain),
                          wscale=float(self.weight_gain))
        y = linear(x, self.weight, None, wscale=float(self.weight_gain))
        return bias_act.bias_act(y, b, act=self.activation)



class SynthesisLayer(torch.nn.Module):
    def __init__(self, in_channels, out_channels, w_dim, resolution, kernel_size=3, up=1, use_noise=True, activation='lrelu',
                 resample_filter=[1, 3, 3, 1], conv_clamp=None, channels_last=False):
        super().__init__()
        if use_noise or conv_clamp is not None or activation != 'lrelu' or kernel_size != 3 or up not in (1, 2):
            raise NotImplementedError('SynthesisLayer: only use_noise=False, conv_clamp=None, lrelu, 3x3, up in {1,2}')
        self.in_channels = in_channels
        self.out_channels = out_channels
        self.w_dim = w_dim
        self.resolution = resolution
        self.up = up
        self.use_noise = use_noise
        self.activation = activation
        self.conv_clamp = conv_clamp
        self.register_buffer('resample_filter', upfirdn2d.setup_filter(resample_filter))
        self.padding = kernel_size // 2
        self.act_gain = bias_act.activation_funcs[activation].def_gain
        self.affine = FullyConnectedLayer(w_dim, in_channels, bias_init=1)
        self.weight = torch.nn.Parameter(torch.randn([out_channels, in_channels, kernel_size, kernel_size]).to(memory_format=torch.channels_last))
        self.bias = torch.nn.Parameter(torch.zeros([out_channels]))

    def forward(self, x, w, noise_mode='none', fused_modconv=False, gain=1):
        if fused_modconv:
            raise NotImplementedError('fused_modconv=True is not used by LayoutDETR (networks_detr.py:261)')
        styles = self.affine(w)
        g = float(self.act_gain * gain)
        if self.up == 1:
            return modconv.modconv3x3(x, self.weight, styles, self.bias, 0.2, g)
        return modconv.modconv3x3_up2(x, self.weight, styles, self.bias, self.resample_filter, 0.2, g)

    def extra_repr(self):
        return (f'in_channels={self.in_channels:d}, out_channels={self.out_channels:d}, w_dim={self.w_dim:d}, '
                f'resolution={self.resolution:d}, up={self.up}, activation={self.activation:s}')


class ToRGBLayer(torch.nn.Module):
    def __init__(self, in_channels, out_channels, w_dim, kernel_size=1, conv_clamp=None, channels_last=False):
        super().__init__()
        if kernel_size != 1 or conv_clamp is not None:
            raise NotImplementedError('ToRGBLayer: only 1x1 without clamping')
        self.in_channels = in_channels
        self.out_channels = out_channels
        self.w_dim = w_dim
        self.conv_clamp = conv_clamp
        self.affine = FullyConnectedLayer(w_dim, in_channels, bias_init=1)
        self.weight = torch.nn.Parameter(torch.randn([out_channels, in_channels, kernel_size, kernel_size]))
        self.bias = torch.nn.Parameter(torch.zeros([out_channels]))
        self.weight_gain = 1 / np.sqrt(in_channels * (kernel_size ** 2))

    def forward(self, x, w, fused_modconv=False):
        styles = self.affine(w) * float(self.weight_gain)
        return modconv.torgb(x, self.weight, styles, self.bias)



class SynthesisBlock(torch.nn.Module):
    def __init__(self, in_channels, out_channels, w_dim, resolution, img_channels, is_last, architecture='skip',
                 resample_filter=[1, 3, 3, 1], conv_clamp=256, use_fp16=False, fp16_channels_last=False,
                 fused_modconv_default=True, **layer_kwargs):
        super().__init__()
        if architecture != 'skip' or use_fp16:
            raise NotImplementedError("SynthesisBlock: only architecture='skip' in fp32")
        self.in_channels = in_channels
        self.w_dim = w_dim
        self.resolution = resolution
        self.img_channels = img_channels
        self.is_last = is_last
        self.architecture = architecture
        self.use_fp16 = use_fp16
        self.channels_last = False
        self.fused_modconv_default = fused_modconv_default
        self.register_buffer('resample_filter', upfirdn2d.setup_filter(resample_filter))
        self.num_conv = 0
        self.num_torgb = 0
        if in_channels == 0:
            self.const = torch.nn.Parameter(torch.randn([out_channels, resolution, resolution]))
        if in_channels != 0:
            self.conv0 = SynthesisLayer(in_channels, out_channels, w_dim=w_dim, resolution=resolution, up=2,
                                        resample_filter=resample_filter, conv_clamp=conv_clamp, **layer_kwargs)
            self.num_conv += 1
        self.conv1 = SynthesisLayer(out_channels, out_channels, w_dim=w_dim, resolution=resolution, conv_clamp=conv_clamp, **layer_kwargs)
        self.num_conv += 1
        self.torgb = ToRGBLayer(out_channels, img_channels, w_dim=w_dim, conv_clamp=conv_clamp)
        self.num_torgb += 1

    def forward(self, x, img, ws, force_fp32=False, fused_modconv=None, update_emas=False, **layer_kwargs):
        w_iter = iter(ws.unbind(dim=1))
        if fused_modconv is None:
            fused_modconv = self.fused_modconv_default
        if fused_modconv == 'inference_only':
            fused_modconv = not self.training
        if self.in_channels == 0:
            x = self.const.permute(1, 2, 0).unsqueeze(0).repeat([ws.shape[0], 1, 1, 1])
            x = self.conv1(x, next(w_iter), fused_modconv=fused_modconv, **layer_kwargs)
        else:
            x = self.conv0(x, next(w_iter), fused_modconv=fused_modconv, **layer_kwargs)
            x = self.conv1(x, next(w_iter), fused_modconv=fused_modconv, **layer_kwargs)
        if img is not None:
            img = upfirdn2d.upsample2d(img.permute(0, 3, 1, 2), self.resample_filter).permute(0, 2, 3, 1)
        y = self.torgb(x, next(w_iter), fused_modconv=fused_modconv)
        img = img + y if img is not None else y
        return x, img



class SynthesisNetwork(torch.nn.Module):
    def __init__(self, w_dim, img_resolution, img_channels, channel_base=32768, channel_max=512, num_fp16_res=4, **block_kwargs):
        assert img_resolution >= 4 and img_resolution & (img_resolution - 1) == 0
        super().__init__()
        if num_fp16_res != 0:
            raise NotImplementedError('fp16 blocks are not used by LayoutDETR (num_fp16_res=0)')
        self.w_dim = w_dim
        self.img_resolution = img_resolution
        self.img_resolution_log2 = int(np.log2(img_resolution))
        self.img_channels = img_channels
        self.num_fp16_res = num_fp16_res
        self.block_resolutions = [2 ** i for i in range(2, self.img_resolution_log2 + 1)]
        channels_dict = {res: min(channel_base // res, channel_max) for res in self.block_resolutions}
        self.num_ws = 0
        for res in self.block_resolutions:
            in_channels = channels_dict[res // 2] if res > 4 else 0
            out_channels = channels_dict[res]
            is_last = (res == self.img_resolution)
            block = SynthesisBlock(in_channels, out_channels, w_dim=w_dim, resolution=res, img_channels=img_channels,
                                   is_last=is_last, use_fp16=False, **block_kwargs)
            self.num_ws += block.num_conv
            if is_last:
                self.num_ws += block.num_torgb
            setattr(self, f'b{res}', block)

    def forward(self, ws, **block_kwargs):
        ws = ws.to(torch.float32)
        x = img = None
        first = 0
        for res in self.block_resolutions:
            block = getattr(self, f'b{res}')
            n = block.num_conv + block.num_torgb
            cur = ws.unsqueeze(1).expand(-1, n, -1) if ws.ndim == 2 else ws[:, first:first + n]
            x, img = block(x, img, cur, **block_kwargs)
            first += block.num_conv
        return img.permute(0, 3, 1, 2)


class DecoderMappingNetwork(torch.nn.Module):
    def __init__(self, z_dim, w_dim, num_ws, num_layers=8, layer_features=None, activation='lrelu', lr_multiplier=0.01,
                 w_avg_beta=0.998):
        super().__init__()
        self.z_dim = z_dim
        self.w_dim = w_dim
        self.num_ws = num_ws
        self.num_layers = num_layers
        self.w_avg_beta = w_avg_beta
        if layer_features is None:
            layer_features = w_dim
        features_list = [z_dim] + [layer_features] * (num_layers - 1) + [w_dim]
        for idx in range(num_layers):
            layer = FullyConnectedLayer(features_list[idx], features_list[idx + 1], activation=activation, lr_multiplier=lr_multiplier)
            setattr(self, f'fc{idx}', layer)
        if num_ws is not None and w_avg_beta is not None:
            self.register_buffer('w_avg', torch.zeros([w_dim]))

    def forward(self, z, truncation_psi=1, truncation_cutoff=None, update_emas=False, broadcast=True):
        w = z.to(torch.float32)
        for idx in range(self.num_layers):
            w = getattr(self, f'fc{idx}')(w)
        if update_emas and self.w_avg_beta is not None:
            self.w_avg.copy_(torch.lerp(w.detach().mean(dim=0), self.w_avg, self.w_avg_beta))
        per_layer = truncation_psi != 1 and self.num_ws is not None and truncation_cutoff is not None
        if truncation_psi != 1 and not per_layer:
            assert self.w_avg_beta is not None
            w = torch.lerp(self.w_avg, w, truncation_psi)
        if self.num_ws is None or (not broadcast and not per_layer):
            return w
        ws = w.unsqueeze(1).repeat([1, self.num_ws, 1])
        if per_layer:
            assert self.w_avg_beta is not None
            head = torch.lerp(self.w_avg, ws[:, :truncation_cutoff], truncation_psi)
            ws = torch.cat([head, ws[:, truncation_cutoff:]], dim=1)
        return ws


class Decoder(torch.nn.Module):
    def __init__(self, z_dim, w_dim, img_resolution, img_channels, use_noise, mapping_kwargs={}, **synthesis_kwargs):
        super().__init__()
        self.z_dim = z_dim
        self.w_dim = w_dim
        self.img_resolution = img_resolution
        self.img_channels = img_channels
        self.synthesis = SynthesisNetwork(w_dim=w_dim, img_resolution=img_resolution, img_channels=img_channels, use_noise=use_noise,
                                          **synthesis_kwargs)
        self.num_ws = self.synthesis.num_ws
        self.mapping = DecoderMappingNetwork(z_dim=z_dim, w_dim=w_dim, num_ws=self.num_ws, **mapping_kwargs)

    def forward(self, z, truncation_psi=1, truncation_cutoff=None, update_emas=False, **synthesis_kwargs):
        ws = self.mapping(z, truncation_psi=truncation_psi, truncation_cutoff=truncation_cutoff, update_emas=update_emas, broadcast=False)
        return self.synthesis(ws, update_emas=update_emas, **synthesis_kwargs)
```

Before: 495.3.

## Fuse StyleGAN2 synthesis backward into a single autograd node with handoff kernels

```diff
diff --git a/include/ldetr_hip.h b/include/ldetr_hip.h
--- a/include/ldetr_hip.h
+++ b/include/ldetr_hip.h
@@ -184,6 +184,9 @@
                         int B, int64_t P, int C, void* stream);
 int ldetr_torgb_bwd_f32(const float* x, const float* dy, const float* w, const float* styles, float* dx, float* dws,
                         float* dbias, int B, int64_t P, int C, void* stream);
+int ldetr_sg2_handoff_f32(const float* dxs, const float* x, const float* dy_rgb, float* dv, const float* s_conv, const float* s_rgb,
+                          const float* w_rgb, const float* bias, const float* demod, float* ds_conv, float* dws_rgb, float* dbias_rgb,
+                          float* dbias, float* ddemod, int B, int64_t P, int C, float alpha, float gain, void* stream);
 
 int ldetr_maxpool3x3s2_fwd_f32(const float* x, float* y, unsigned char* idx, int N, int H, int W, int C, void* stream);
 int ldetr_maxpool3x3s2_bwd_f32(const float* dy, const unsigned char* idx, float* dx, int N, int H, int W, int C,
diff --git a/layoutdetr_amd/_lib.py b/layoutdetr_amd/_lib.py
--- a/layoutdetr_amd/_lib.py
+++ b/layoutdetr_amd/_lib.py
@@ -147,6 +147,7 @@
     'ldetr_masked_mse_fwd_f32': [_P, _P, _P, _L, _I, _I, _P, _P],
     'ldetr_masked_mse_bwd_f32': [_P, _P, _P, _L, _I, _I, _P, _P, _P, _P],
     'ldetr_torgb_bwd_finish_f32': [_P, _P, _P, _I, _I, _P, _P, _P],
+    'ldetr_sg2_handoff_f32': [_P, _P, _P, _P, _P, _P, _P, _P, _P, _P, _P, _P, _P, _P, _I, _L, _I, _F, _F, _P],
     'ldetr_gemm_pair_f32': [_P, _P, _P],
     'ldetr_gemm_pair_is_single_launch': [_P, _P],
     'ldetr_demod_fwd_f32': [_P, _L, _L, _L, _L, _P, _P, _P, _I, _I, _I, _I, _I, _F, _P],
diff --git a/layoutdetr_amd/build.py b/layoutdetr_amd/build.py
--- a/layoutdetr_amd/build.py
+++ b/layoutdetr_amd/build.py
@@ -18,7 +18,7 @@
 
 FLAGS = ([] if os.environ.get('LDETR_TILE_TRACE') else ['-DLDETR_TILE_TRACE=0']) + (['-DP3_TRACE'] if os.environ.get('LDETR_P3_TRACE') else []) + ['-O3', '-std=c++17', '-fPIC', f'--offload-arch={ARCH}', '-munsafe-fp-atomics', '-fno-gpu-rdc',
          '-Wno-unused-result', '-Rpass-analysis=kernel-resource-usage']
-NO_SCRATCH = ('wgrad_c32_3x3_kernel', 'gemm_f32_kernel', 'gemm_small_kernel', 'attn_fwd_kernel', 'attn_fwd_wide_kernel', 'attn_bwd_kernel', 'ffn_fwd_kernel', 'ffn_bwd_kernel', 'conv3x3_c32_kernel', 'mha_small_fwd_kernel', 'mha_cross_fwd_kernel', 'mha_small_bwd_kernel', 'mha_cross_bwd_kernel', 'wgrad_multi_kernel', 'ln_fwd_kernel', 'ln_bwd_kernel', 'p3_nt_kernel', 'p3_tn_kernel', 'p3_c3_kernel', 'p3_bwd_pair', 'layoutnet_features_kernel', 'layoutnet_forward_kernel', 'feature_stats_f64_kernel', 'layout_finish_kernel', 'layout_raster_kernel', 'page_blur_kernel', 'page_edge_kernel', 'patch_resize_kernel')
+NO_SCRATCH = ('wgrad_c32_3x3_kernel', 'gemm_f32_kernel', 'gemm_small_kernel', 'attn_fwd_kernel', 'attn_fwd_wide_kernel', 'attn_bwd_kernel', 'ffn_fwd_kernel', 'ffn_bwd_kernel', 'conv3x3_c32_kernel', 'mha_small_fwd_kernel', 'mha_cross_fwd_kernel', 'mha_small_bwd_kernel', 'mha_cross_bwd_kernel', 'wgrad_multi_kernel', 'ln_fwd_kernel', 'ln_bwd_kernel', 'p3_nt_kernel', 'p3_tn_kernel', 'p3_c3_kernel', 'p3_bwd_pair', 'layoutnet_features_kernel', 'layoutnet_forward_kernel', 'feature_stats_f64_kernel', 'layout_finish_kernel', 'layout_raster_kernel', 'page_blur_kernel', 'page_edge_kernel', 'patch_resize_kernel', 'sg2_handoff_kernel')
 
 
 def _hipcc():
diff --git a/layoutdetr_amd/csrc/misc_ops.hip b/layoutdetr_amd/csrc/misc_ops.hip
--- a/layoutdetr_amd/csrc/misc_ops.hip
+++ b/layoutdetr_amd/csrc/misc_ops.hip
@@ -1,5 +1,6 @@
 #include "ldetr_common.hpp"
 #include "../../include/ldetr_hip.h"
+#include <type_traits>
 
 namespace ldetr {
 
@@ -104,46 +105,63 @@
     }
 }
 
-__global__ __launch_bounds__(256) void rr_finish_kernel(RRParams p, int chunks, int segs) {
+enum { RR_MAX_PLANES = 6 };
+struct RRFinish {
+    float* red[RR_MAX_PLANES]; long bs[RR_MAX_PLANES];
+    const float* part; int B, C;
+};
+
+__global__ __launch_bounds__(256) void rr_finish_kernel(RRFinish f, int chunks, int segs) {
     __shared__ float sh[256];
     const int which = blockIdx.z / segs, seg = blockIdx.z % segs;
-    float* red = which ? p.red2 : p.red1;
-    const long bs = which ? p.red2_bs : p.red1_bs;
+    float* red = nullptr; long bs = 0;
+#pragma unroll
+    for (int i = 0; i < RR_MAX_PLANES; i++) if (which == i) { red = f.red[i]; bs = f.bs[i]; }
     if (!red) return;
     const bool shared_by_batch = bs == 0;
     if (shared_by_batch && blockIdx.y > 0) return;
     const int c = blockIdx.x * 64 + (threadIdx.x & 63), lane = threadIdx.x >> 6;
-    const long nblk = (long)chunks * p.B;
-    const float* part = p.part + (which ? nblk * p.C : 0);
+    const long nblk = (long)chunks * f.B;
+    const float* part = f.part + (long)which * nblk * f.C;
     const long first = shared_by_batch ? 0 : (long)blockIdx.y * chunks, count = shared_by_batch ? nblk : chunks;
     const long per = (count + segs - 1) / segs, i0 = seg * per, i1 = min(count, i0 + per);
     float acc = 0.f;
-    if (c < p.C) {
+    if (c < f.C) {
 #pragma unroll 4
-        for (long i = i0 + lane; i < i1; i += 4) acc += part[(first + i) * p.C + c];
+        for (long i = i0 + lane; i < i1; i += 4) acc += part[(first + i) * f.C + c];
     }
     sh[threadIdx.x] = acc;
     __syncthreads();
-    if (lane == 0 && c < p.C && i0 < i1) {
+    if (lane == 0 && c < f.C && i0 < i1) {
         acc += sh[threadIdx.x + 64] + sh[threadIdx.x + 128] + sh[threadIdx.x + 192];
         float* d = red + (shared_by_batch ? 0 : (long)blockIdx.y * bs) + c;
         if (segs > 1) atomicAdd(d, acc); else *d += acc;
     }
 }
 
-static int launch_rr(RRParams& p, hipStream_t st) {
-    const int C4 = p.C / 4;
+static dim3 rr_grid(int B, long P, int C, int* rows_pb_out) {
+    const int C4 = C / 4;
     const int TQ = C4 < 256 ? C4 : 256;
     const int RL = 256 / TQ;
     static const long target = 2048;
-    const long groups = (long)p.B * cdiv(C4, TQ);
+    const long groups = (long)B * cdiv(C4, TQ);
     long chunks = target / groups; if (chunks < 1) chunks = 1;
-    long rows_pb = (p.P + chunks - 1) / chunks;
+    long rows_pb = (P + chunks - 1) / chunks;
     const long min_rows = (long)RL * 4;
     if (rows_pb < min_rows) rows_pb = min_rows;
     rows_pb = (rows_pb + RL - 1) / RL * RL;
-    p.rows_pb = (int)rows_pb;
-    dim3 grid((unsigned)((p.P + rows_pb - 1) / rows_pb), p.B, cdiv(C4, TQ));
+    *rows_pb_out = (int)rows_pb;
+    return dim3((unsigned)((P + rows_pb - 1) / rows_pb), B, cdiv(C4, TQ));
+}
+
+static int launch_rr_finish(const RRFinish& f, int planes, int chunks, long sharers, hipStream_t st) {
+    int segs = (int)(sharers / 32); if (segs < 1) segs = 1; if (segs > 16) segs = 16;
+    hipLaunchKernelGGL(rr_finish_kernel, dim3(cdiv(f.C, 64), f.B, planes * segs), 256, 0, st, f, chunks, segs);
+    return check_launch("rowreduce_finish");
+}
+
+static int launch_rr(RRParams& p, hipStream_t st) {
+    const dim3 grid = rr_grid(p.B, p.P, p.C, &p.rows_pb);
     const long nblk = (long)grid.x * grid.y;
     const long sharers = p.red1 && p.red1_bs == 0 ? nblk : (long)grid.x;
     p.part = (p.red1 || p.red2) && sharers > 32 ? scratch_alloc((size_t)nblk * p.C * sizeof(float) * (p.red2 ? 2 : 1)) : nullptr;
@@ -151,9 +169,9 @@
     else if (p.mode == RR_ACTGRAD) hipLaunchKernelGGL(rowreduce_kernel<RR_ACTGRAD>, grid, 256, 0, st, p);
     else hipLaunchKernelGGL(rowreduce_kernel<RR_MULRED>, grid, 256, 0, st, p);
     int rc = check_launch("rowreduce"); if (rc || !p.part) return rc;
-    int segs = (int)(sharers / 32); if (segs < 1) segs = 1; if (segs > 16) segs = 16;
-    hipLaunchKernelGGL(rr_finish_kernel, dim3(cdiv(p.C, 64), p.B, (p.red2 ? 2 : 1) * segs), 256, 0, st, p, (int)grid.x, segs);
-    return check_launch("rowreduce_finish");
+    RRFinish f; memset(&f, 0, sizeof(f));
+    f.red[0] = p.red1; f.bs[0] = p.red1_bs; f.red[1] = p.red2; f.bs[1] = p.red2_bs; f.part = p.part; f.B = p.B; f.C = p.C;
+    return launch_rr_finish(f, p.red2 ? 2 : 1, (int)grid.x, sharers, st);
 }
 
 struct PoolParams {
@@ -305,6 +323,173 @@
     }
 }
 
+struct HandoffParams {
+    const float* dxs; const float* x; const float* dy; float* dv;
+    const float* s_conv; const float* s_rgb; const float* w_rgb; const float* bias; const float* demod;
+    float* ds_conv; float* dws; float* dbias_rgb; float* dbias; float* ddemod;
+    float* part;
+    long P; int B, C, rows_pb;
+    float gp, gn;
+};
+
+static __device__ __forceinline__ void f4_fma(float4& acc, float s, const float4& v) {
+    acc.x += s * v.x; acc.y += s * v.y; acc.z += s * v.z; acc.w += s * v.w;
+}
+static __device__ __forceinline__ void f4_add(float4& acc, const float4& v) { acc.x += v.x; acc.y += v.y; acc.z += v.z; acc.w += v.w; }
+
+template <bool CONV, bool RGB>
+__global__ __launch_bounds__(256) __attribute__((amdgpu_waves_per_eu(CONV && RGB ? 4 : 5))) void sg2_handoff_kernel(HandoffParams p) {
+    __shared__ float4 sh[3][256];
+    __shared__ float4 shw[3][256];
+    const int C4 = p.C >> 2;
+    const int TQ = C4 < 256 ? C4 : 256;
+    const int RL = 256 / TQ;
+    const int tx = threadIdx.x % TQ, ty = threadIdx.x / TQ;
+    const int cq = blockIdx.z * TQ + tx;
+    const int b = blockIdx.y;
+    const bool active = (ty < RL) && (cq < C4);
+    const bool dd = p.ddemod != nullptr;
+    if (RGB) {
+        if (active && ty == 0) {
+            const int c = cq << 2;
+            const float4 sr = *reinterpret_cast<const float4*>(p.s_rgb + (long)b * p.C + c);
+#pragma unroll
+            for (int k = 0; k < 3; k++) {
+                const float4 w = *reinterpret_cast<const float4*>(p.w_rgb + (long)k * p.C + c);
+                shw[k][tx] = make_float4(sr.x * w.x, sr.y * w.y, sr.z * w.z, sr.w * w.w);
+            }
+        }
+        __syncthreads();
+    }
+    const float4 zero = make_float4(0.f, 0.f, 0.f, 0.f);
+    float4 rs = zero, rb = zero, rd = zero, a0 = zero, a1 = zero, a2 = zero;
+    float db0 = 0.f, db1 = 0.f, db2 = 0.f;
+    if (active) {
+        const int c = cq << 2;
+        float4 sc = zero;
+        if (CONV) sc = *reinterpret_cast<const float4*>(p.s_conv + (long)b * p.C + c);
+        const float gp = p.gp, gn = p.gn;
+        const float ip = 1.f / gp, in = (gn != 0.f) ? 1.f / gn : 0.f;
+        const long r0 = (long)blockIdx.x * p.rows_pb;
+        const int nrows = (int)(min(p.P, r0 + p.rows_pb) - r0);
+        const long base = ((long)b * p.P + r0) * p.C;
+        const char* xb = reinterpret_cast<const char*>(p.x + base);
+        const char* ab = CONV ? reinterpret_cast<const char*>(p.dxs + base) : nullptr;
+        const char* yb = RGB ? reinterpret_cast<const char*>(p.dy + ((long)b * p.P + r0) * 3) : nullptr;
+        char* ob = reinterpret_cast<char*>(p.dv + base);
+        const unsigned rowb = (unsigned)p.C * 4u, cb = (unsigned)c * 4u;
+        auto trip = [&](int r, auto un) {
+            constexpr int UN = decltype(un)::value;
+            float4 av[UN], xv[UN];
+            float d0[UN], d1[UN], d2[UN];
+#pragma unroll
+            for (int u = 0; u < UN; u++) {
+                const unsigned off = (unsigned)r * rowb + cb, yo = (unsigned)r * 12u;
+                const size_t ub = (size_t)(u * RL) * rowb, uy = (size_t)(u * RL) * 12u;
+                if (CONV) av[u] = *reinterpret_cast<const float4*>(ab + ub + off);
+                xv[u] = *reinterpret_cast<const float4*>(xb + ub + off);
+                if (RGB) {
+                    d0[u] = *reinterpret_cast<const float*>(yb + uy + yo); d1[u] = *reinterpret_cast<const float*>(yb + uy + 4 + yo);
+                    d2[u] = *reinterpret_cast<const float*>(yb + uy + 8 + yo);
+                }
+            }
+#pragma unroll
+            for (int u = 0; u < UN; u++) {
+                __builtin_amdgcn_sched_barrier(0);
+                const float4& x = xv[u];
+                float4 g = zero;
+                if (RGB) {
+                    int wi = tx;
+                    asm volatile("" : "+v"(wi));
+                    f4_fma(g, d0[u], shw[0][wi]); f4_fma(g, d1[u], shw[1][wi]); f4_fma(g, d2[u], shw[2][wi]);
+                    f4_fma(a0, d0[u], x); f4_fma(a1, d1[u], x); f4_fma(a2, d2[u], x);
+                    db0 += d0[u]; db1 += d1[u]; db2 += d2[u];
+                }
+                if (CONV) {
+                    const float4& a = av[u];
+                    g.x += a.x * sc.x; g.y += a.y * sc.y; g.z += a.z * sc.z; g.w += a.w * sc.w;
+                    rs.x += a.x * x.x; rs.y += a.y * x.y; rs.z += a.z * x.z; rs.w += a.w * x.w;
+                }
+                float4 dv;
+                dv.x = x.x > 0.f ? g.x * gp : g.x * gn; dv.y = x.y > 0.f ? g.y * gp : g.y * gn;
+                dv.z = x.z > 0.f ? g.z * gp : g.z * gn; dv.w = x.w > 0.f ? g.w * gp : g.w * gn;
+                *reinterpret_cast<float4*>(ob + (size_t)(u * RL) * rowb + ((unsigned)r * rowb + cb)) = dv;
+                f4_add(rb, dv);
+                rd.x += dv.x * (x.x > 0.f ? x.x * ip : x.x * in); rd.y += dv.y * (x.y > 0.f ? x.y * ip : x.y * in);
+                rd.z += dv.z * (x.z > 0.f ? x.z * ip : x.z * in); rd.w += dv.w * (x.w > 0.f ? x.w * ip : x.w * in);
+            }
+        };
+        int r = ty;
+#pragma nounroll
+        for (; r + 3 * RL < nrows; r += 4 * RL) trip(r, std::integral_constant<int, 4>());
+#pragma nounroll
+        for (; r < nrows; r += RL) trip(r, std::integral_constant<int, 1>());
+    }
+    const bool lead = active && ty == 0;
+    const int c = cq << 2;
+    const long nblk = (long)gridDim.x * gridDim.y, blk = (long)blockIdx.y * gridDim.x + blockIdx.x;
+    auto emit = [&](const float4& v, int plane, float* red, long bs) {
+        if (p.part) { *reinterpret_cast<float4*>(p.part + ((long)plane * nblk + blk) * p.C + c) = v; return; }
+        float* d = red + (long)b * bs + c;
+        atomicAdd(d, v.x); atomicAdd(d + 1, v.y); atomicAdd(d + 2, v.z); atomicAdd(d + 3, v.w);
+    };
+    if (RGB) {
+        sh[0][threadIdx.x] = a0; sh[1][threadIdx.x] = a1; sh[2][threadIdx.x] = a2;
+        __syncthreads();
+        if (lead) {
+            for (int j = 1; j < RL; j++) { f4_add(a0, sh[0][j * TQ + tx]); f4_add(a1, sh[1][j * TQ + tx]); f4_add(a2, sh[2][j * TQ + tx]); }
+            const int pl = CONV ? 1 : 0;
+            emit(a0, pl, p.dws, 3L * p.C); emit(a1, pl + 1, p.dws + p.C, 3L * p.C); emit(a2, pl + 2, p.dws + 2 * p.C, 3L * p.C);
+        }
+        __syncthreads();
+    }
+    sh[0][threadIdx.x] = rs; sh[1][threadIdx.x] = rb; sh[2][threadIdx.x] = rd;
+    __syncthreads();
+    if (lead) {
+        for (int j = 1; j < RL; j++) { f4_add(rs, sh[0][j * TQ + tx]); f4_add(rb, sh[1][j * TQ + tx]); f4_add(rd, sh[2][j * TQ + tx]); }
+        const int pl = (CONV ? 1 : 0) + (RGB ? 3 : 0);
+        if (CONV) emit(rs, 0, p.ds_conv, p.C);
+        emit(rb, pl, p.dbias, 0);
+        if (dd) {
+            const float4 dmv = *reinterpret_cast<const float4*>(p.demod + (long)b * p.C + c);
+            const float4 cv = p.bias ? *reinterpret_cast<const float4*>(p.bias + c) : make_float4(0.f, 0.f, 0.f, 0.f);
+            rd.x = (rd.x - cv.x * rb.x) / dmv.x; rd.y = (rd.y - cv.y * rb.y) / dmv.y;
+            rd.z = (rd.z - cv.z * rb.z) / dmv.z; rd.w = (rd.w - cv.w * rb.w) / dmv.w;
+            emit(rd, pl + 1, p.ddemod, p.C);
+        }
+    }
+    if (RGB && blockIdx.z == 0) {
+        __syncthreads();
+        float* f = reinterpret_cast<float*>(&sh[0][0]);
+        if (tx == 0 && ty < RL) { f[ty * 3] = db0; f[ty * 3 + 1] = db1; f[ty * 3 + 2] = db2; }
+        __syncthreads();
+        if (threadIdx.x < 3) {
+            float t = 0.f;
+            for (int j = 0; j < RL; j++) t += f[j * 3 + threadIdx.x];
+            atomicAdd(p.dbias_rgb + threadIdx.x, t);
+        }
+    }
+}
+
+template <bool CONV, bool RGB>
+static int launch_handoff(HandoffParams& p, hipStream_t st) {
+    const dim3 grid = rr_grid(p.B, p.P, p.C, &p.rows_pb);
+    LDETR_CHECK((long)p.rows_pb * p.C < (1L << 30), "sg2_handoff: a row chunk of %d x %d floats exceeds the kernel's 32-bit offsets", p.rows_pb, p.C);
+    const long nblk = (long)grid.x * grid.y;
+    const int planes = (CONV ? 1 : 0) + (RGB ? 3 : 0) + 1 + (p.ddemod ? 1 : 0);
+    p.part = nblk > 32 ? scratch_alloc((size_t)planes * nblk * p.C * sizeof(float)) : nullptr;
+    hipLaunchKernelGGL((sg2_handoff_kernel<CONV, RGB>), grid, 256, 0, st, p);
+    int rc = check_launch("sg2_handoff"); if (rc || !p.part) return rc;
+    RRFinish f; memset(&f, 0, sizeof(f));
+    int i = 0;
+    if (CONV) { f.red[i] = p.ds_conv; f.bs[i++] = p.C; }
+    if (RGB) for (int k = 0; k < 3; k++) { f.red[i] = p.dws + (long)k * p.C; f.bs[i++] = 3L * p.C; }
+    f.red[i] = p.dbias; f.bs[i++] = 0;
+    if (p.ddemod) { f.red[i] = p.ddemod; f.bs[i++] = p.C; }
+    f.part = p.part; f.B = p.B; f.C = p.C;
+    return launch_rr_finish(f, planes, (int)grid.x, nblk, st);
+}
+
 }
 
 using namespace ldetr;
@@ -458,6 +643,29 @@
     return check_launch("torgb_bwd");
 }
 
+extern "C" int ldetr_sg2_handoff_f32(const float* dxs, const float* x, const float* dy_rgb, float* dv, const float* s_conv, const float* s_rgb,
+                                     const float* w_rgb, const float* bias, const float* demod, float* ds_conv, float* dws_rgb,
+                                     float* dbias_rgb, float* dbias, float* ddemod, int B, int64_t P, int C, float alpha, float gain,
+                                     void* stream) {
+    LDETR_CHECK(x && dv && dbias, "sg2_handoff: x, dv and dbias are required");
+    LDETR_CHECK(dxs || dy_rgb, "sg2_handoff: neither a conv gradient nor an rgb gradient");
+    LDETR_CHECK(!dxs || (s_conv && ds_conv), "sg2_handoff: dxs needs s_conv and ds_conv");
+    LDETR_CHECK(!dy_rgb || (s_rgb && w_rgb && dws_rgb && dbias_rgb), "sg2_handoff: dy_rgb needs s_rgb, w_rgb, dws_rgb and dbias_rgb");
+    LDETR_CHECK(!ddemod || demod, "sg2_handoff: ddemod needs demod");
+    LDETR_CHECK(C % 4 == 0 && C > 0 && B > 0 && P >= 0, "sg2_handoff: C must be a positive multiple of 4, B > 0 (got B %d, C %d)", B, C);
+    LDETR_CHECK((((uintptr_t)dxs | (uintptr_t)x | (uintptr_t)dv | (uintptr_t)s_conv | (uintptr_t)s_rgb | (uintptr_t)w_rgb | (uintptr_t)bias |
+                  (uintptr_t)demod) & 15) == 0, "sg2_handoff: buffers must be 16-byte aligned");
+    if (P == 0) return LDETR_OK;
+    HandoffParams p; memset(&p, 0, sizeof(p));
+    p.dxs = dxs; p.x = x; p.dy = dy_rgb; p.dv = dv; p.s_conv = s_conv; p.s_rgb = s_rgb; p.w_rgb = w_rgb; p.bias = bias; p.demod = demod;
+    p.ds_conv = ds_conv; p.dws = dws_rgb; p.dbias_rgb = dbias_rgb; p.dbias = dbias; p.ddemod = ddemod;
+    p.B = B; p.P = P; p.C = C; p.gp = gain; p.gn = gain * alpha;
+    hipStream_t st = (hipStream_t)stream;
+    if (dxs && dy_rgb) return launch_handoff<true, true>(p, st);
+    if (dxs) return launch_handoff<true, false>(p, st);
+    return launch_handoff<false, true>(p, st);
+}
+
 extern "C" int ldetr_torgb_bwd_finish_f32(const float* dws, const float* s, const float* w, int B, int C, float* dw, float* ds, void* stream) {
     LDETR_CHECK(dws && s && w && dw && ds && B > 0 && C > 0, "torgb_bwd_finish: bad arguments");
     const int n = (B > 3 ? B : 3) * C;
diff --git a/layoutdetr_amd/hip/modconv.py b/layoutdetr_amd/hip/modconv.py
--- a/layoutdetr_amd/hip/modconv.py
+++ b/layoutdetr_amd/hip/modconv.py
@@ -24,20 +24,122 @@
     return x, dv, s, d
 
 
+def _wgrad_target(wparam, O, KH, KW, I, device):
+    gw = core.flat_grad(wparam)
+    if gw is not None and gw.permute(0, 2, 3, 1).is_contiguous():
+        return gw.permute(0, 2, 3, 1), 1
+    return torch.empty((O, KH, KW, I), device=device, dtype=torch.float32), 0
+
+
+def conv_fwd(x, w, s, d, b, pad, act_alpha, act_gain):
+    B, H, W, I = x.shape
+    O, KH, KW, _ = w.shape
+    OH, OW = H + 2 * pad - KH + 1, W + 2 * pad - KW + 1
+    y = torch.empty((B, OH, OW, O), device=x.device, dtype=torch.float32)
+    xt = core.tensor4_nhwc(x)
+    ep = core.epilogue(samp_scale=d, col_bias=b, act=ACT_LRELU, act_alpha=act_alpha, act_gain=act_gain)
+    core.engine_call('ldetr_conv2d_fwd_f32', 2.0 * B * OH * OW * O * KH * KW * I, lambda: core.check(core.lib().ldetr_conv2d_fwd_f32(core.ptr(x), ctypes.byref(xt), core.ptr(w), O, KH, KW, 1, pad, core.ptr(y), O,
+                                               OH, OW, core.ptr(s), s.stride(0), ctypes.byref(ep), core.stream()), 'modconv_fwd'), operands=(x, y, w))
+    return y
+
+
+def conv_bwd_data(dv, w, d, B, H, W, pad):
+    O, KH, KW, I = w.shape
+    _, OH, OW, _ = dv.shape
+    dvt = core.tensor4_nhwc(dv)
+    dxs = torch.empty((B, H, W, I), device=dv.device, dtype=torch.float32)
+    core.engine_call('ldetr_conv2d_bwd_data_f32', 2.0 * B * OH * OW * O * KH * KW * I, lambda: core.check(core.lib().ldetr_conv2d_bwd_data_f32(core.ptr(dv), ctypes.byref(dvt), core.ptr(w), I, KH, KW, 1, pad,
+                                                    core.ptr(dxs), I, H, W, core.ptr(d), d.stride(0), None, core.stream()),
+               'modconv_bwd_data'), operands=(dv, dxs, w))
+    return dxs
+
+
+def conv_bwd_weight(x, dv, w, s, d, wparam, pad):
+    B, H, W, I = x.shape
+    O, KH, KW, _ = w.shape
+    _, OH, OW, _ = dv.shape
+    dw_ohwi, acc = _wgrad_target(wparam, O, KH, KW, I, dv.device)
+    sk = 0
+    xw, dvw, sw, dw_ = _prescaled_for_wgrad(x, dv, s, d, B, H)
+    xwt, dvwt = core.tensor4_nhwc(xw), core.tensor4_nhwc(dvw)
+    core.engine_call('ldetr_conv2d_bwd_weight_f32', 2.0 * B * OH * OW * O * KH * KW * I, lambda: core.check(core.lib().ldetr_conv2d_bwd_weight_f32(core.ptr(xw), ctypes.byref(xwt), core.ptr(dvw), ctypes.byref(dvwt),
+                                                      core.ptr(dw_ohwi), KH, KW, 1, pad, sk, core.ptr(sw), sw.stride(0) if sw is not None else 0,
+                                                      core.ptr(dw_), dw_.stride(0) if dw_ is not None else 0, acc, core.stream()), 'modconv_bwd_weight'), operands=(x, dv, dw_ohwi))
+    return None if acc else _grad_to_oihw(dw_ohwi)
+
+
+def up_fwd(x, w, s, d, b, f, act_alpha, act_gain):
+    B, H, W, I = x.shape
+    O, KH, KW, _ = w.shape
+    UH, UW = (H - 1) * 2 + KH, (W - 1) * 2 + KW
+    ud = torch.empty((B, UH, UW, O), device=x.device, dtype=torch.float32)
+    xt = core.tensor4_nhwc(x)
+    ep = core.epilogue(samp_scale=d)
+    core.engine_call('ldetr_conv_transpose2d_fwd_f32', 2.0 * B * H * W * O * KH * KW * I, lambda: core.check(core.lib().ldetr_conv_transpose2d_fwd_f32(core.ptr(x), ctypes.byref(xt), core.ptr(w), O, KH, KW, 2, 0, core.ptr(ud),
+                                                         O, UH, UW, core.ptr(s), s.stride(0), ctypes.byref(ep), core.stream()),
+               'modconv_up_fwd'), operands=(x, ud, w))
+    y = _up._kernel_call(ud.permute(0, 3, 1, 2), f, 1, 1, 1, 1, 1, 1, 1, 1, False, 4.0, act_bias=b,
+                         act=(act_alpha, act_gain)).permute(0, 2, 3, 1)
+    return ud, y
+
+
+def up_fir_adjoint(dv, f):
+    return _up._kernel_call(dv.permute(0, 3, 1, 2), f, 1, 1, 1, 1, 2, 2, 2, 2, True, 4.0).permute(0, 2, 3, 1)
+
+
+def up_bwd_data(dud, w, d, B, H, W):
+    O, KH, KW, I = w.shape
+    dudt = core.tensor4_nhwc(dud)
+    dxs = torch.empty((B, H, W, I), device=dud.device, dtype=torch.float32)
+    core.engine_call('ldetr_conv_transpose2d_bwd_data_f32', 2.0 * B * H * W * O * KH * KW * I, lambda: core.check(core.lib().ldetr_conv_transpose2d_bwd_data_f32(core.ptr(dud), ctypes.byref(dudt), core.ptr(w), I, KH, KW, 2, 0,
+                                                              core.ptr(dxs), I, H, W, core.ptr(d), d.stride(0), None,
+                                                              core.stream()), 'modconv_up_bwd_data'), operands=(dud, dxs, w))
+    return dxs
+
+
+def up_bwd_weight(x, dud, w, s, d, wparam):
+    B, H, W, I = x.shape
+    O, KH, KW, _ = w.shape
+    dw_ohwi, acc = _wgrad_target(wparam, O, KH, KW, I, dud.device)
+    sk = 0
+    xw, dudw, sw, dw_ = _prescaled_for_wgrad(x, dud, s, d, B, H)
+    xwt, dudwt = core.tensor4_nhwc(xw), core.tensor4_nhwc(dudw)
+    core.engine_call('ldetr_conv_transpose2d_bwd_weight_f32', 2.0 * B * H * W * O * KH * KW * I, lambda: core.check(core.lib().ldetr_conv_transpose2d_bwd_weight_f32(core.ptr(xw), ctypes.byref(xwt), core.ptr(dudw), ctypes.byref(dudwt),
+                                                                core.ptr(dw_ohwi), KH, KW, 2, 0, sk, core.ptr(sw), sw.stride(0) if sw is not None else 0,
+                                                                core.ptr(dw_), dw_.stride(0) if dw_ is not None else 0, acc, core.stream()), 'modconv_up_bwd_weight'), operands=(x, dud, dw_ohwi))
+    return None if acc else _grad_to_oihw(dw_ohwi)
+
+
+def torgb_fwd(x, w, s, b):
+    B, H, W, C = x.shape
+    O = w.shape[0]
+    y = torch.empty((B, H, W, O), device=x.device, dtype=torch.float32)
+    c4 = C // 4
+    if O == 3 and C % 4 == 0 and C <= 512 and (c4 & (c4 - 1)) == 0 and s.stride(0) == C:
+        core.check(core.lib().ldetr_torgb_fwd_f32(core.ptr(x), core.ptr(w), core.ptr(s), core.ptr(b), core.ptr(y), B, H * W, C, core.stream()), 'torgb_fwd')
+    else:
+        xt = core.tensor4_nhwc(x)
+        ep = core.epilogue(col_bias=b)
+        core.engine_call('ldetr_conv2d_fwd_f32', 2.0 * B * H * W * O * C, lambda: core.check(core.lib().ldetr_conv2d_fwd_f32(core.ptr(x), ctypes.byref(xt), core.ptr(w), O, 1, 1, 1, 0, core.ptr(y), O, H, W,
+                                                   core.ptr(s), s.stride(0), ctypes.byref(ep), core.stream()), 'torgb_fwd'), operands=(x, y, w))
+    return y
+
+
+def torgb_grad_targets(wparam, bparam, O, C, device):
+    gw, gb = core.flat_grad(wparam), core.flat_grad(bparam)
+    gw = gw.reshape(O, C) if (gw is not None and gw.is_contiguous()) else None
+    dbias = gb if gb is not None else torch.zeros(O, device=device, dtype=torch.float32)
+    dw = gw if gw is not None else torch.zeros((O, C), device=device, dtype=torch.float32)
+    return dw, dbias, gw is not None, gb is not None
+
+
 class _ModConvFn(torch.autograd.Function):
 
     @staticmethod
     def forward(ctx, x, weight, styles, dcoefs, bias, pad, act_alpha, act_gain):
         core.require_gpu(x, weight, styles, dcoefs, bias)
         x = core.f32c(x); w = core.f32c(weight_ohwi(weight)); s = core.f32c(styles); d = core.f32c(dcoefs); b = core.f32c(bias)
-        B, H, W, I = x.shape
-        O, KH, KW, _ = w.shape
-        OH, OW = H + 2 * pad - KH + 1, W + 2 * pad - KW + 1
-        y = torch.empty((B, OH, OW, O), device=x.device, dtype=torch.float32)
-        xt = core.tensor4_nhwc(x)
-        ep = core.epilogue(samp_scale=d, col_bias=b, act=ACT_LRELU, act_alpha=act_alpha, act_gain=act_gain)
-        core.engine_call('ldetr_conv2d_fwd_f32', 2.0 * B * OH * OW * O * KH * KW * I, lambda: core.check(core.lib().ldetr_conv2d_fwd_f32(core.ptr(x), ctypes.byref(xt), core.ptr(w), O, KH, KW, 1, pad, core.ptr(y), O,
-                                                   OH, OW, core.ptr(s), s.stride(0), ctypes.byref(ep), core.stream()), 'modconv_fwd'), operands=(x, y, w))
+        y = conv_fwd(x, w, s, d, b, pad, act_alpha, act_gain)
         ctx.save_for_backward(x, w, s, d, b, y)
         ctx.cfg = (pad, act_alpha, act_gain)
         ctx.params = (weight, bias)
@@ -55,28 +157,12 @@
         dv2, dbias, ddemod = act_backward(dy.reshape(-1, O), y.reshape(-1, O), ACT_LRELU, act_alpha, act_gain, True,
                                           bias=b, demod=d, want_ddemod=True, B=B, dbias_out=core.flat_grad(bparam))
         dv = dv2.reshape(B, OH, OW, O)
-        dvt = core.tensor4_nhwc(dv)
         dx = dw = ds = None
         if ctx.needs_input_grad[0] or ctx.needs_input_grad[2]:
-            dxs = torch.empty((B, H, W, I), device=dy.device, dtype=torch.float32)
-            core.engine_call('ldetr_conv2d_bwd_data_f32', 2.0 * B * OH * OW * O * KH * KW * I, lambda: core.check(core.lib().ldetr_conv2d_bwd_data_f32(core.ptr(dv), ctypes.byref(dvt), core.ptr(w), I, KH, KW, 1, pad,
-                                                            core.ptr(dxs), I, H, W, core.ptr(d), d.stride(0), None, core.stream()),
-                       'modconv_bwd_data'), operands=(dv, dxs, w))
+            dxs = conv_bwd_data(dv, w, d, B, H, W, pad)
             dx, ds = _mul_reduce(dxs, x, s, B, H * W, I)
         if ctx.needs_input_grad[1]:
-            gw = core.flat_grad(wparam)
-            acc = 0
-            if gw is not None and gw.permute(0, 2, 3, 1).is_contiguous():
-                dw_ohwi, acc = gw.permute(0, 2, 3, 1), 1
-            else:
-                dw_ohwi = torch.empty((O, KH, KW, I), device=dy.device, dtype=torch.float32)
-            sk = 0
-            xw, dvw, sw, dw_ = _prescaled_for_wgrad(x, dv, s, d, B, H)
-            xwt, dvwt = core.tensor4_nhwc(xw), core.tensor4_nhwc(dvw)
-            core.engine_call('ldetr_conv2d_bwd_weight_f32', 2.0 * B * OH * OW * O * KH * KW * I, lambda: core.check(core.lib().ldetr_conv2d_bwd_weight_f32(core.ptr(xw), ctypes.byref(xwt), core.ptr(dvw), ctypes.byref(dvwt),
-                                                              core.ptr(dw_ohwi), KH, KW, 1, pad, sk, core.ptr(sw), sw.stride(0) if sw is not None else 0,
-                                                              core.ptr(dw_), dw_.stride(0) if dw_ is not None else 0, acc, core.stream()), 'modconv_bwd_weight'), operands=(x, dv, dw_ohwi))
-            dw = None if acc else _grad_to_oihw(dw_ohwi)
+            dw = conv_bwd_weight(x, dv, w, s, d, wparam, pad)
         return dx, dw, ds, ddemod, dbias, None, None, None
 
 
@@ -86,59 +172,30 @@
     def forward(ctx, x, weight, styles, dcoefs, bias, f, act_alpha, act_gain):
         core.require_gpu(x, weight, styles, dcoefs, bias, f)
         x = core.f32c(x); w = core.f32c(weight_ohwi(weight)); s = core.f32c(styles); d = core.f32c(dcoefs); b = core.f32c(bias)
-        B, H, W, I = x.shape
-        O, KH, KW, _ = w.shape
-        UH, UW = (H - 1) * 2 + KH, (W - 1) * 2 + KW
-        ud = torch.empty((B, UH, UW, O), device=x.device, dtype=torch.float32)
-        xt = core.tensor4_nhwc(x)
-        ep = core.epilogue(samp_scale=d)
-        core.engine_call('ldetr_conv_transpose2d_fwd_f32', 2.0 * B * H * W * O * KH * KW * I, lambda: core.check(core.lib().ldetr_conv_transpose2d_fwd_f32(core.ptr(x), ctypes.byref(xt), core.ptr(w), O, KH, KW, 2, 0, core.ptr(ud),
-                                                             O, UH, UW, core.ptr(s), s.stride(0), ctypes.byref(ep), core.stream()),
-                   'modconv_up_fwd'), operands=(x, ud, w))
-        y = _up._kernel_call(ud.permute(0, 3, 1, 2), f, 1, 1, 1, 1, 1, 1, 1, 1, False, 4.0, act_bias=b,
-                             act=(act_alpha, act_gain)).permute(0, 2, 3, 1)
-        ctx.save_for_backward(x, w, s, d, b, f, ud, y)
+        _, y = up_fwd(x, w, s, d, b, f, act_alpha, act_gain)
+        ctx.save_for_backward(x, w, s, d, b, f, y)
         ctx.cfg = (act_alpha, act_gain)
         ctx.params = (weight, bias)
         return y
 
     @staticmethod
     def backward(ctx, dy):
-        x, w, s, d, b, f, ud, y = ctx.saved_tensors
+        x, w, s, d, b, f, y = ctx.saved_tensors
         act_alpha, act_gain = ctx.cfg
         B, H, W, I = x.shape
         O, KH, KW, _ = w.shape
-        _, UH, UW, _ = ud.shape
         dy = core.f32c(dy)
         wparam, bparam = ctx.params
-        dv2, dbias, _ = act_backward(dy.reshape(-1, O), y.reshape(-1, O), ACT_LRELU, act_alpha, act_gain, True,
-                                     dbias_out=core.flat_grad(bparam))
+        dv2, dbias, ddemod = act_backward(dy.reshape(-1, O), y.reshape(-1, O), ACT_LRELU, act_alpha, act_gain, True,
+                                          bias=b, demod=d, want_ddemod=True, B=B, dbias_out=core.flat_grad(bparam))
         dv = dv2.reshape(y.shape)
-        dud = _up._kernel_call(dv.permute(0, 3, 1, 2), f, 1, 1, 1, 1, 2, 2, 2, 2, True, 4.0).permute(0, 2, 3, 1)
-        _, dd_num = _mul_reduce(dud, ud, None, B, UH * UW, O, want_out=False)
-        ddemod = dd_num / d
-        dudt = core.tensor4_nhwc(dud)
+        dud = up_fir_adjoint(dv, f)
         dx = dw = ds = None
         if ctx.needs_input_grad[0] or ctx.needs_input_grad[2]:
-            dxs = torch.empty((B, H, W, I), device=dy.device, dtype=torch.float32)
-            core.engine_call('ldetr_conv_transpose2d_bwd_data_f32', 2.0 * B * H * W * O * KH * KW * I, lambda: core.check(core.lib().ldetr_conv_transpose2d_bwd_data_f32(core.ptr(dud), ctypes.byref(dudt), core.ptr(w), I, KH, KW, 2, 0,
-                                                                      core.ptr(dxs), I, H, W, core.ptr(d), d.stride(0), None,
-                                                                      core.stream()), 'modconv_up_bwd_data'), operands=(dud, dxs, w))
+            dxs = up_bwd_data(dud, w, d, B, H, W)
             dx, ds = _mul_reduce(dxs, x, s, B, H * W, I)
         if ctx.needs_input_grad[1]:
-            gw = core.flat_grad(wparam)
-            acc = 0
-            if gw is not None and gw.permute(0, 2, 3, 1).is_contiguous():
-                dw_ohwi, acc = gw.permute(0, 2, 3, 1), 1
-            else:
-                dw_ohwi = torch.empty((O, KH, KW, I), device=dy.device, dtype=torch.float32)
-            sk = 0
-            xw, dudw, sw, dw_ = _prescaled_for_wgrad(x, dud, s, d, B, H)
-            xwt, dudwt = core.tensor4_nhwc(xw), core.tensor4_nhwc(dudw)
-            core.engine_call('ldetr_conv_transpose2d_bwd_weight_f32', 2.0 * B * H * W * O * KH * KW * I, lambda: core.check(core.lib().ldetr_conv_transpose2d_bwd_weight_f32(core.ptr(xw), ctypes.byref(xwt), core.ptr(dudw), ctypes.byref(dudwt),
-                                                                        core.ptr(dw_ohwi), KH, KW, 2, 0, sk, core.ptr(sw), sw.stride(0) if sw is not None else 0,
-                                                                        core.ptr(dw_), dw_.stride(0) if dw_ is not None else 0, acc, core.stream()), 'modconv_up_bwd_weight'), operands=(x, dud, dw_ohwi))
-            dw = None if acc else _grad_to_oihw(dw_ohwi)
+            dw = up_bwd_weight(x, dud, w, s, d, wparam)
         return dx, dw, ds, ddemod, dbias, None, None, None
 
 
@@ -149,17 +206,7 @@
         core.require_gpu(x, weight, styles, bias)
         x = core.f32c(x); s = core.f32c(styles); b = core.f32c(bias)
         w = core.f32c(weight.reshape(weight.shape[0], -1))
-        B, H, W, C = x.shape
-        O = w.shape[0]
-        y = torch.empty((B, H, W, O), device=x.device, dtype=torch.float32)
-        c4 = C // 4
-        if O == 3 and C % 4 == 0 and C <= 512 and (c4 & (c4 - 1)) == 0 and s.stride(0) == C:
-            core.check(core.lib().ldetr_torgb_fwd_f32(core.ptr(x), core.ptr(w), core.ptr(s), core.ptr(b), core.ptr(y), B, H * W, C, core.stream()), 'torgb_fwd')
-        else:
-            xt = core.tensor4_nhwc(x)
-            ep = core.epilogue(col_bias=b)
-            core.engine_call('ldetr_conv2d_fwd_f32', 2.0 * B * H * W * O * C, lambda: core.check(core.lib().ldetr_conv2d_fwd_f32(core.ptr(x), ctypes.byref(xt), core.ptr(w), O, 1, 1, 1, 0, core.ptr(y), O, H, W,
-                                                       core.ptr(s), s.stride(0), ctypes.byref(ep), core.stream()), 'torgb_fwd'), operands=(x, y, w))
+        y = torgb_fwd(x, w, s, b)
         ctx.save_for_backward(x, w, s)
         ctx.wshape = weight.shape
         ctx.params = (weight, bias)
@@ -176,15 +223,12 @@
         dx = torch.empty_like(x)
         dws = core.zeros((B, O, C), x.device)
         wparam, bparam = ctx.params
-        gw, gb = core.flat_grad(wparam), core.flat_grad(bparam)
-        gw = gw.reshape(O, C) if (gw is not None and gw.is_contiguous()) else None
-        dbias = gb if gb is not None else torch.zeros(O, device=x.device, dtype=torch.float32)
-        dw = gw if gw is not None else torch.zeros((O, C), device=x.device, dtype=torch.float32)
+        dw, dbias, w_flat, b_flat = torgb_grad_targets(wparam, bparam, O, C, x.device)
         ds = torch.empty((B, C), device=x.device, dtype=torch.float32)
         core.check(core.lib().ldetr_torgb_bwd_f32(core.ptr(x), core.ptr(dy), core.ptr(w), core.ptr(s), core.ptr(dx), core.ptr(dws),
                                                   core.ptr(dbias), B, H * W, C, core.stream()), 'torgb_bwd')
         core.check(core.lib().ldetr_torgb_bwd_finish_f32(core.ptr(dws), core.ptr(s), core.ptr(w), B, C, core.ptr(dw), core.ptr(ds), core.stream()), 'torgb_bwd_finish')
-        return dx, (None if gw is not None else dw.reshape(ctx.wshape)), ds, (None if gb is not None else dbias)
+        return dx, (None if w_flat else dw.reshape(ctx.wshape)), ds, (None if b_flat else dbias)
 
 
 class _DemodFn(torch.autograd.Function):
diff --git a/layoutdetr_amd/hip/sg2_chain.py b/layoutdetr_amd/hip/sg2_chain.py
--- /dev/null
+++ b/layoutdetr_amd/hip/sg2_chain.py
@@ -0,0 +1,155 @@
+import torch
+
+from . import core, modconv
+from .conv import weight_ohwi
+from ..torch_utils.ops import upfirdn2d as _up
+
+ENABLED = core.knob('SG2_CHAIN', 1) != 0
+ACT_ALPHA = 0.2
+NODE_RUNS = [0]
+
+
+class Block(object):
+
+    def __init__(self, has_conv0, gains, params):
+        self.has_conv0 = has_conv0
+        self.gains = gains
+        self.params = params
+
+
+def _handoff(dxs, x, dy_rgb, s_conv, rgb, bias, demod, dbias, gain):
+    B, H, W, C = x.shape
+    dev = x.device
+    dv = dxs if dxs is not None else torch.empty_like(x)
+    ds_conv = core.zeros((B, C), dev) if dxs is not None else None
+    dws = core.zeros((B, 3, C), dev) if dy_rgb is not None else None
+    ddemod = core.zeros((B, C), dev)
+    s_rgb, w_rgb, dbias_rgb = rgb if dy_rgb is not None else (None, None, None)
+    core.check(core.lib().ldetr_sg2_handoff_f32(core.ptr(dxs), core.ptr(x), core.ptr(dy_rgb), core.ptr(dv), core.ptr(s_conv), core.ptr(s_rgb), core.ptr(w_rgb),
+                                                core.ptr(bias), core.ptr(demod), core.ptr(ds_conv), core.ptr(dws), core.ptr(dbias_rgb), core.ptr(dbias),
+                                                core.ptr(ddemod), B, H * W, C, ACT_ALPHA, gain, core.stream()), 'sg2_handoff')
+    return dv, ds_conv, dws, ddemod
+
+
+def _bias_target(bparam, C, device):
+    gb = core.flat_grad(bparam)
+    if gb is not None:
+        return gb, True
+    return torch.zeros(C, device=device, dtype=torch.float32), False
+
+
+class _SynthesisFn(torch.autograd.Function):
+
+    @staticmethod
+    def forward(ctx, blocks, const, f, *tensors):
+        core.require_gpu(const, f, *tensors)
+        keep = any(ctx.needs_input_grad)
+        it = iter(tensors)
+        saved, layout = [const, f], []
+        x = img = None
+        B = tensors[2].shape[0]
+        for blk in blocks:
+            entry = {}
+            if blk.has_conv0:
+                w, b, s, d = [next(it) for _ in range(4)]
+                w = core.f32c(weight_ohwi(w)); b = core.f32c(b); s = core.f32c(s); d = core.f32c(d)
+                _, x0 = modconv.up_fwd(x, w, s, d, b, f, ACT_ALPHA, blk.gains[0])
+                entry['conv0'] = (w, b, s, d, x0)
+                x = x0
+            else:
+                x = core.f32c(const).permute(1, 2, 0).unsqueeze(0).repeat([B, 1, 1, 1])
+                entry['xin'] = (x,)
+            w, b, s, d = [next(it) for _ in range(4)]
+            w = core.f32c(weight_ohwi(w)); b = core.f32c(b); s = core.f32c(s); d = core.f32c(d)
+            x = modconv.conv_fwd(x, w, s, d, b, w.shape[1] // 2, ACT_ALPHA, blk.gains[1])
+            entry['conv1'] = (w, b, s, d, x)
+            if img is not None:
+                img = _up._kernel_call(img.permute(0, 3, 1, 2), f, 2, 2, 1, 1, 2, 1, 2, 1, False, 4.0).permute(0, 2, 3, 1)
+            w, b, s = [next(it) for _ in range(3)]
+            ctx_wshape = w.shape
+            w = core.f32c(w.reshape(w.shape[0], -1)); b = core.f32c(b); s = core.f32c(s)
+            if w.shape[0] != 3:
+                raise NotImplementedError('the synthesis node is specialised for 3 colour channels')
+            y = modconv.torgb_fwd(x, w, s, b)
+            img = img + y if img is not None else y
+            entry['torgb'] = (w, s)
+            entry['rgb_wshape'] = ctx_wshape
+            if keep:
+                rec = {}
+                for k in ('conv0', 'xin', 'conv1', 'torgb'):
+                    if k in entry:
+                        rec[k] = (len(saved), len(entry[k]))
+                        saved += list(entry[k])
+                rec['rgb_wshape'] = ctx_wshape
+                layout.append(rec)
+        if keep:
+            ctx.save_for_backward(*saved)
+            ctx.blocks, ctx.layout = blocks, layout
+        return img
+
+    @staticmethod
+    def backward(ctx, dimg):
+        saved = ctx.saved_tensors
+        const, f = saved[0], saved[1]
+        blocks, layout = ctx.blocks, ctx.layout
+        need = ctx.needs_input_grad[3:]
+        get = lambda rec, k: saved[rec[k][0]:rec[k][0] + rec[k][1]]
+        dimg = core.f32c(dimg)
+        dev = dimg.device
+        grads = [None] * len(need)
+        first, n = [], 0
+        for blk in blocks:
+            first.append(n)
+            n += 11 if blk.has_conv0 else 7
+        dxs_next = s_next = dconst = None
+        for i in reversed(range(len(blocks))):
+            blk, rec = blocks[i], layout[i]
+            o = first[i] + (4 if blk.has_conv0 else 0)
+            w1, b1, s1, d1, x1 = get(rec, 'conv1')
+            wr, sr = get(rec, 'torgb')
+            B, H, W, C = x1.shape
+            (w1p, b1p), (wrp, brp) = blk.params['conv1'], blk.params['torgb']
+            dw_rgb, dbias_rgb, wr_flat, br_flat = modconv.torgb_grad_targets(wrp, brp, 3, C, dev)
+            db1, b1_flat = _bias_target(b1p, C, dev)
+            dv1, ds_next, dws, dd1 = _handoff(dxs_next, x1, dimg, s_next, (sr, wr, dbias_rgb), b1, d1, db1, blk.gains[1])
+            ds_rgb = torch.empty((B, C), device=dev, dtype=torch.float32)
+            core.check(core.lib().ldetr_torgb_bwd_finish_f32(core.ptr(dws), core.ptr(sr), core.ptr(wr), B, C, core.ptr(dw_rgb), core.ptr(ds_rgb), core.stream()),
+                       'torgb_bwd_finish')
+            if i + 1 < len(blocks):
+                grads[first[i + 1] + 2] = ds_next
+            grads[o + 4] = None if wr_flat else dw_rgb.reshape(rec['rgb_wshape'])
+            grads[o + 5] = None if br_flat else dbias_rgb
+            grads[o + 6] = ds_rgb
+            grads[o + 1] = None if b1_flat else db1
+            grads[o + 3] = dd1
+            xin = get(rec, 'conv0')[4] if blk.has_conv0 else get(rec, 'xin')[0]
+            pad = w1.shape[1] // 2
+            dxs1 = modconv.conv_bwd_data(dv1, w1, d1, B, xin.shape[1], xin.shape[2], pad)
+            if need[o]:
+                grads[o] = modconv.conv_bwd_weight(xin, dv1, w1, s1, d1, w1p, pad)
+            if not blk.has_conv0:
+                dx, ds1 = modconv._mul_reduce(dxs1, xin, s1, B, xin.shape[1] * xin.shape[2], xin.shape[3])
+                grads[o + 2] = ds1
+                if ctx.needs_input_grad[1]:
+                    dconst = dx.sum(0).permute(2, 0, 1)
+                break
+            w0, b0, s0, d0, x0 = get(rec, 'conv0')
+            w0p, b0p = blk.params['conv0']
+            db0, b0_flat = _bias_target(b0p, C, dev)
+            dv0, ds1, _, dd0 = _handoff(dxs1, x0, None, s1, None, b0, d0, db0, blk.gains[0])
+            grads[o + 2] = ds1
+            grads[first[i] + 1] = None if b0_flat else db0
+            grads[first[i] + 3] = dd0
+            dud = modconv.up_fir_adjoint(dv0, f)
+            xprev = get(layout[i - 1], 'conv1')[4]
+            dxs_next = modconv.up_bwd_data(dud, w0, d0, B, xprev.shape[1], xprev.shape[2])
+            s_next = s0
+            if need[first[i]]:
+                grads[first[i]] = modconv.up_bwd_weight(xprev, dud, w0, s0, d0, w0p)
+            dimg = _up._kernel_call(dimg.permute(0, 3, 1, 2), f, 1, 1, 2, 2, 1, 1, 1, 1, True, 4.0).permute(0, 2, 3, 1)
+        return (None, dconst, None) + tuple(grads)
+
+
+def run(blocks, const, f, tensors):
+    NODE_RUNS[0] += 1
+    return _SynthesisFn.apply(blocks, const, f, *tensors)
diff --git a/layoutdetr_amd/training/networks_stylegan2.py b/layoutdetr_amd/training/networks_stylegan2.py
--- a/layoutdetr_amd/training/networks_stylegan2.py
+++ b/layoutdetr_amd/training/networks_stylegan2.py
@@ -3,7 +3,7 @@
 import numpy as np
 import torch
 
-from ..hip import core, modconv
+from ..hip import core, modconv, sg2_chain
 from ..hip.linear import linear
 from ..torch_utils.ops import bias_act, upfirdn2d
 
@@ -174,6 +174,8 @@
 
     def forward(self, ws, **block_kwargs):
         ws = ws.to(torch.float32)
+        if sg2_chain.ENABLED and not (set(block_kwargs) - {'update_emas', 'noise_mode', 'force_fp32'}):
+            return self._forward_node(ws)
         x = img = None
         first = 0
         for res in self.block_resolutions:
@@ -182,6 +184,29 @@
             cur = ws.unsqueeze(1).expand(-1, n, -1) if ws.ndim == 2 else ws[:, first:first + n]
             x, img = block(x, img, cur, **block_kwargs)
             first += block.num_conv
+        return img.permute(0, 3, 1, 2)
+
+
+    def _forward_node(self, ws):
+        blocks, tensors = [], []
+        first = 0
+        for res in self.block_resolutions:
+            block = getattr(self, f'b{res}')
+            n = block.num_conv + block.num_torgb
+            w_iter = iter([ws] * n if ws.ndim == 2 else ws[:, first:first + n].unbind(dim=1))
+            layers = ([block.conv0] if block.in_channels != 0 else []) + [block.conv1]
+            for layer in layers:
+                styles = layer.affine(next(w_iter))
+                tensors += [layer.weight, layer.bias, styles, modconv.demod_coefs(layer.weight, styles)]
+            tensors += [block.torgb.weight, block.torgb.bias, block.torgb.affine(next(w_iter)) * float(block.torgb.weight_gain)]
+            gains = (float(block.conv0.act_gain) if block.in_channels != 0 else None, float(block.conv1.act_gain))
+            params = {'conv1': (block.conv1.weight, block.conv1.bias), 'torgb': (block.torgb.weight, block.torgb.bias)}
+            if block.in_channels != 0:
+                params['conv0'] = (block.conv0.weight, block.conv0.bias)
+            blocks.append(sg2_chain.Block(block.in_channels != 0, gains, params))
+            first += block.num_conv
+        b4 = getattr(self, f'b{self.block_resolutions[0]}')
+        img = sg2_chain.run(blocks, b4.const, b4.resample_filter, tensors)
         return img.permute(0, 3, 1, 2)
 
 
```

New measurement: 501.3, median of 6. +1.2%, better.
